# Beryl2000/SE-UNet-AirSeg

Hardware: AMD Instinct MI355X
Metric: voxels/sec SE-UNet fwd+bwd, 128^3 patch (higher is better)
Workload: dtype bf16

## Files before the change

### include/seunet_hip.h

```cpp
#ifndef SEUNET_HIP_H
#define SEUNET_HIP_H
#include <stddef.h>

#ifdef __cplusplus
extern "C" {
#endif

#ifndef SEUNET_F32
#define SEUNET_F32 0
#define SEUNET_BF16 1
#define SEUNET_F16 2
#endif
#define SEUNET_CONV_MFMA 0
#define SEUNET_CONV_NAIVE 1
#define SEUNET_CONV_MARCH 2
#define SEUNET_CONV_TILED 3

typedef void* seunet_stream_t;
typedef struct seunet_dims { int n, d, h, w; } seunet_dims;

int seunet_version(void);
const char* seunet_last_error(void);
int seunet_init(int device);

int seunet_pack_cl(int dtype, const float* in_ncdhw, int c, void* out_cl, int c_pad, seunet_dims dims, seunet_stream_t s);
int seunet_unpack_cl(int dtype, const void* in_cl, int c, float* out_ncdhw, seunet_dims dims, seunet_stream_t s);

size_t seunet_conv_wpack_bytes(int dtype, int taps, int cin, int cout);
int seunet_conv_pack_weights(int dtype, const float* w, int taps, int cin, int cout, int transpose_flip, void* wpack, seunet_stream_t s);
int seunet_conv_stats_slots(int impl, int taps, int dilation, seunet_dims dims);
int seunet_conv3d_fwd(int dtype, int impl, int taps, int dilation, int nsrc, const void* const* src, const int* src_c,
                      int cin, const void* weights, int transpose_flip, const float* bias, int ndst, void* const* dst,
                      const int* dst_c, const int* dst_accumulate, double* stats_partial, seunet_dims dims, seunet_stream_t s);
int seunet_conv3d_stream_supported(int dtype, int dilation, int src_c, int dst_c);
size_t seunet_conv3d_stream_wpack_bytes(int src_c);
int seunet_conv3d_stream_slots(int dilation, seunet_dims dims);
int seunet_conv3d_stream_pack(int dtype, const float* w, int cin_w, int cout_w, int transpose_flip, int src_c, int dst_c, void* wpack,
                              seunet_stream_t s);
int seunet_conv3d_stream(int dtype, int dilation, const void* src, int src_c, const void* wpack, const float* bias, void* dst, int dst_c,
                         int dst_accumulate, double* stats_partial, seunet_dims dims, seunet_stream_t s);
int seunet_conv3d_march_supported(int dtype, int dilation, int nsrc, const int* src_c, int ndst, const int* dst_c);
size_t seunet_conv3d_march_wpack_bytes(int cin, int cout);
int seunet_conv3d_march_slots(int dilation, int cin, int cout, seunet_dims dims);
int seunet_conv3d_march_pack(int dtype, const float* w, int cin_w, int cout_w, int transpose_flip, int cin, int cout, void* wpack,
                             seunet_stream_t s);
int seunet_conv3d_march(int dtype, int dilation, int nsrc, const void* const* src, const int* src_c, const void* wpack, const float* bias,
                        int ndst, void* const* dst, const int* dst_c, const int* dst_accumulate, double* stats_partial, seunet_dims dims,
                        seunet_stream_t s);
int seunet_conv3d_wgrad_stream_supported(int dtype, int dilation, int x_c, int dy_c);
size_t seunet_conv3d_wgrad_stream_workspace_bytes(int x_c, int dy_c, int dilation, seunet_dims dims);
int seunet_conv3d_wgrad_stream(int dtype, int dilation, const void* x, int x_c, int cin, const void* dy, int dy_c, int cout, float* dw,
                               void* workspace, size_t workspace_bytes, seunet_dims dims, seunet_stream_t s);
size_t seunet_conv3d_wgrad_workspace_bytes(int taps, int cin, int cout);
int seunet_conv3d_wgrad(int dtype, int impl, int taps, int dilation, int nsrc, const void* const* src, const int* src_c,
                        int cin, const void* dy, int cout, float* dw, void* workspace, size_t workspace_bytes,
                        seunet_dims dims, seunet_stream_t s);

int seunet_epilogue_slots(seunet_dims dims);
int seunet_channel_stats(int dtype, const void* t, int c, double* partial, seunet_dims dims, seunet_stream_t s);
int seunet_stats_finalize(const double* partial, int slots, int c, int n, long long count, float eps, int mode,
                          float* out_a, float* out_b, seunet_stream_t s);

int seunet_gate_epilogue_fwd(int dtype, const void* raw, const float* mean, const float* rstd, int c, const float* w_se,
                             const float* w_se2, const float* w_side, const float* b_side, float slope, void* e_out,
                             float* side_out, float* level_map, int level_accumulate, const float* head_w,
                             const float* drop, int drop_stride, seunet_dims dims, seunet_stream_t s);
int seunet_gate_epilogue_bwd(int dtype, const void* raw, const float* mean, const float* rstd, int c, const float* w_se,
                             const float* w_se2, const float* w_side, const float* b_side, float slope, const void* g_e,
                             const float* g_side, const float* g_level, const float* head_w, const float* drop,
                             int drop_stride, const float* m1, const float* m2, void* draw_out, double* stat_partial,
                             float* pgrad_partial, seunet_dims dims, seunet_stream_t s);
int seunet_pgrad_reduce(const float* pgrad_partial, int records, int c, float* dw_se, float* dw_se2, float* dw_side,
                        float* db_side, float* dhead_w, seunet_stream_t s);
int seunet_gate_bwd_finalize(const double* stat_partial, int slots, int c, int n, long long count, float* m1, float* m2,
                             const float* pgrad_partial, int records, float* dw_se, float* dw_se2, float* dw_side,
                             float* db_side, float* dhead_w, seunet_stream_t s);

int seunet_cat_epilogue_fwd(int dtype, const void* raw, const float* mean, const float* rstd, const void* raw2,
                            const float* mean2, const float* rstd2, int c, float slope, void* out, seunet_dims dims,
                            seunet_stream_t s);
int seunet_cat_epilogue_bwd(int dtype, const void* g_out, const void* raw, const float* mean, const float* rstd,
                            const void* raw2, const float* mean2, const float* rstd2, int c, float slope,
                            const float* m1, const float* m2, const float* m1b, const float* m2b, void* dx, void* dx2,
                            double* stat_partial, double* stat_partial2, seunet_dims dims, seunet_stream_t s);

int seunet_xbranch_moment_slots(seunet_dims dims);
int seunet_xbranch_moments(int dtype, const void* x_in, double* partial , seunet_dims dims, seunet_stream_t s);
int seunet_xbranch_stats(const double* partial, int slots, const float* w2, int c, int in_channel, int n, long long count,
                         float eps, float* mean2, float* rstd2, double* moments_out , seunet_stream_t s);
int seunet_cat_epilogue_fwd_x(int dtype, const void* raw, const float* mean, const float* rstd, const void* x_in,
                              const float* w2, int in_channel, const float* mean2, const float* rstd2, int c, float slope,
                              void* out, seunet_dims dims, seunet_stream_t s);
int seunet_cat_epilogue_bwd_x(int dtype, const void* g_out, const void* raw, const float* mean, const float* rstd,
                              const void* x_in, const float* w2, int in_channel, const float* mean2, const float* rstd2,
                              int c, float slope, const float* m1, const float* m2, const float* m1b, const float* m2b,
                              void* dx, double* stat_partial, double* stat_partial2, double* xw_partial, seunet_dims dims,
                              seunet_stream_t s);
int seunet_cat_epilogue_fwd_x_pool(int dtype, const void* raw, const float* mean, const float* rstd, const void* x_in,
                                   const float* w2, int in_channel, const float* mean2, const float* rstd2, int c, float slope,
                                   void* out, void* pooled, unsigned int* argmax, seunet_dims dims, seunet_stream_t s);
int seunet_cat_epilogue_bwd_x_pool(int dtype, const void* g_out, const void* raw, const float* mean, const float* rstd,
                                   const void* x_in, const float* w2, int in_channel, const float* mean2, const float* rstd2,
                                   int c, float slope, const float* m1, const float* m2, const float* m1b, const float* m2b,
                                   void* dx, double* stat_partial, double* stat_partial2, double* xw_partial,
                                   const unsigned int* pool_argmax, const void* pool_g, seunet_dims dims, seunet_stream_t s);
int seunet_cat_xgrad_finalize(const double* xw_partial, const double* stat_partial2, int slots, const double* moments,
                              const float* w2, int c, int in_channel, int n, float eps, float* dw, seunet_stream_t s);

int seunet_maxpool_fwd(int dtype, const void* in, int c, void* out, seunet_dims in_dims, seunet_stream_t s);
int seunet_maxpool_bwd(int dtype, const void* in, const void* g_out, int c, void* g_in, int accumulate,
                       seunet_dims in_dims, seunet_stream_t s);
int seunet_upsample2_fwd(int dtype, const void* in, int c, void* out, seunet_dims in_dims, seunet_stream_t s);
int seunet_upsample2_bwd(int dtype, const void* g_out, int c, void* g_in, int accumulate, seunet_dims in_dims,
                         seunet_stream_t s);
int seunet_side_upsample(const float* side, int c, int scale, float* out_ncdhw, int c_total, int c_off,
                         seunet_dims low_dims, seunet_stream_t s);

int seunet_head_fwd(const float* const* level_maps, int nlevels, const float* bias, float* pred, seunet_dims dims,
                    seunet_stream_t s);
size_t seunet_head_bwd_tmp_floats(seunet_dims dims);
int seunet_head_bwd(const float* g_pred, float* const* g_levels, int nlevels, float* tmp, float* g_bias,
                    seunet_dims dims, seunet_stream_t s);

#define SEUNET_LOSS_DICE 1
#define SEUNET_LOSS_GUL 2
#define SEUNET_LOSS_ATR 4
int seunet_loss_partial_floats(void);
int seunet_loss_sums(const float* pred, int apply_sigmoid, const float* target, const float* weight, const float* skel,
                     long long n, float* partial, double* sums, int terms, seunet_stream_t s);
int seunet_loss_value(const double* sums0, double c_dice0, double c_gul0, double c_atr0, const double* sums1, double c_dice1,
                      double c_gul1, double c_atr1, float* value, seunet_stream_t s);
int seunet_loss_grad(const float* pred, int apply_sigmoid, const float* target, const float* weight, const float* skel,
                     long long n, const double* sums, float c_dice, float c_gul, float c_atr, float g_scale,
                     const float* g_scale_dev, float* g_pred, seunet_stream_t s);

int seunet_loss_sample_partial_floats(int batch);
int seunet_loss_sums_per_sample(const float* pred, int apply_sigmoid, const float* target, const float* weight, const float* skel,
                                int batch, long long n_per_sample, float* partial, double* sums, int terms, seunet_stream_t s);
int seunet_loss_sample_values(const double* sums, int batch, double c_dice, double c_gul, double c_atr, float* values,
                              seunet_stream_t s);

int seunet_pool_select(const float* new_keys, int batch, float* keys, long long* seq, long long* state, int capacity, int* slots_out,
                       seunet_stream_t s);
int seunet_pool_scatter(const int* slots_dev, int batch, int capacity, long long voxels, const float* data, const float* label,
                        const float* weight, const float* skel, float* pool_data, unsigned char* pool_label, float* pool_weight,
                        unsigned char* pool_skel, seunet_stream_t s);
int seunet_pool_gather(const int* slots_host, int n, int capacity, long long voxels, const float* pool_data,
                       const unsigned char* pool_label, const float* pool_weight, const unsigned char* pool_skel, float* data_out,
                       float* label_out, float* weight_out, float* skel_out, seunet_stream_t s);

int seunet_adamw_step(float* const* params, const float* const* grads, float* const* exp_avg, float* const* exp_avg_sq,
                      const long long* counts, int n_tensors, double lr, double beta1, double beta2, double eps,
                      double weight_decay, int step, int maximize, seunet_stream_t s);

#define SEUNET_IMG_I16 0
#define SEUNET_IMG_F32 1
#define SEUNET_W_F16 0
#define SEUNET_W_F32 1
#define SEUNET_W_F64 2
int seunet_crop_batch(const void* img, int img_dtype, const unsigned char* label, const void* weight, int weight_dtype,
                      const unsigned char* skeleton, int d, int h, int w, int cube, int ncrop, const int* starts, const int* aug,
                      double weight_exponent, int f64_math, float* data_out, float* label_out, float* weight_out, float* skel_out,
                      seunet_stream_t s);
int seunet_hu_two_channel(const void* img, int img_dtype, long long nvox, int f64_math, float* out, seunet_stream_t s);

int seunet_window_gather(const float* volume, int c, int x, int y, int z, int cube, int nwin, const int* starts, float* out,
                         seunet_stream_t s);
int seunet_window_accumulate(const float* logits, int apply_sigmoid, int nwin, const int* starts, int cube, double* acc, int x, int y,
                             int z, seunet_stream_t s);
int seunet_window_finalize(const double* acc, int x, int y, int z, int cube, int nx, const int* xs, int ny, const int* ys, int nz,
                           const int* zs, int dup0, double* out, seunet_stream_t s);

#define SEUNET_DTI_F64 0
#define SEUNET_DTI_F32 1
size_t seunet_dti_workspace_bytes(int h, int w, int z);
int seunet_dti(const double* pred, int h, int w, int z, double h_thresh, double l_thresh, int pred_dtype, unsigned char* out,
               void* workspace, size_t workspace_bytes, seunet_stream_t s);

#define SEUNET_CC_EVALUATION 0
#define SEUNET_CC_MAXIMUM_3D 1
#define SEUNET_CC_LARGEST_FILLED 2
size_t seunet_cc_workspace_bytes(int h, int w, int z);
int seunet_largest_component(const unsigned char* volume, int h, int w, int z, int rule, unsigned char* out, int* status_dev,
                             void* workspace, size_t workspace_bytes, seunet_stream_t s);
size_t seunet_metric_out_bytes(int nbins);
int seunet_metric_sums(const unsigned char* pred, const unsigned char* label, const unsigned char* skeleton, const int* parsing,
                       long long n, int nbins, void* out, size_t out_bytes, seunet_stream_t s);

size_t seunet_edt_workspace_bytes(int n0, int n1, int n2);
int seunet_edt(const unsigned char* volume, int n0, int n1, int n2, int* sqdist, double* dist, int* indices, int* status_dev,
               void* workspace, size_t workspace_bytes, seunet_stream_t s);
int seunet_mask_bits(const unsigned char* mask, long long n, unsigned long long* bits, seunet_stream_t s);
int seunet_hard_mining_masks(const unsigned char* label, const unsigned char* skeleton, const unsigned char* pred, int n0, int n1,
                             int n2, unsigned long long* skeleton_bits, unsigned long long* small_bits, seunet_stream_t s);
size_t seunet_lib_weight_workspace_bytes(int n0, int n1, int n2);
int seunet_lib_weight(const unsigned char* label, int n0, int n1, int n2, const float* table, void* out, void* workspace,
                      size_t workspace_bytes, seunet_stream_t s);
size_t seunet_break_weight_workspace_bytes(int n0, int n1, int n2);
int seunet_break_weight(const unsigned char* label, const unsigned char* pred, const unsigned char* skeleton, int n0, int n1, int n2,
                        void* w_br, unsigned char* br_skel, int* status_dev, void* workspace, size_t workspace_bytes,
                        seunet_stream_t s);

size_t seunet_skeleton_workspace_bytes(int n0, int n1, int n2);
int seunet_skeletonize(const unsigned char* volume, int n0, int n1, int n2, unsigned char* out, int* passes_dev, void* workspace,
                       size_t workspace_bytes, seunet_stream_t s);

size_t seunet_skeleton_branches_workspace_bytes(int n0, int n1, int n2);
int seunet_skeleton_branches(const unsigned char* skeleton, int n0, int n1, int n2, int min_voxels, int* cd, unsigned char* skeleton_parse,
                             int* num_dev, void* workspace, size_t workspace_bytes, seunet_stream_t s);
size_t seunet_parse_assign_workspace_bytes(int n0, int n1, int n2);
int seunet_parse_assign(const unsigned char* skeleton_parse, const int* cd, const unsigned char* label, int n0, int n1, int n2,
                        int* parsing, int* status_dev, void* workspace, size_t workspace_bytes, seunet_stream_t s);
int seunet_label_stats_max_num(void);
int seunet_label_stats(const int* parsing, int n0, int n1, int n2, int num, unsigned int* counts, unsigned long long* adjacency_bits,
                       int* status_dev, seunet_stream_t s);
int seunet_relabel(const int* parsing, long long n, const int* lut, int nlut, int* out, seunet_stream_t s);

#define SEUNET_MORPH_DILATE 0
#define SEUNET_MORPH_ERODE_BORDER0 1
#define SEUNET_MORPH_ERODE_BORDER1 2
#define SEUNET_MORPH_CLOSE 3
size_t seunet_binary_morph_workspace_bytes(int n0, int n1, int n2);
int seunet_binary_morph(const unsigned char* volume, int n0, int n1, int n2, int op, unsigned char* out, void* workspace,
                        size_t workspace_bytes, seunet_stream_t s);
int seunet_fill_holes(const unsigned char* volume, int n0, int n1, int n2, unsigned char* out, void* workspace, size_t workspace_bytes,
                      seunet_stream_t s);
int seunet_slice_moments(const unsigned char* mask, int n0, int n1, int n2, int k, unsigned long long* out_dev, seunet_stream_t s);
int seunet_scatter_labels(const long long* lin_index_dev, const int* value_dev, long long m, long long n, int* cd,
                          unsigned char* skeleton_parse, int* status_dev, seunet_stream_t s);

size_t seunet_mesh_workspace_bytes(int n0, int n1, int n2);
int seunet_mesh_count(const unsigned char* volume, int n0, int n1, int n2, long long* nverts, long long* nfaces, void* workspace,
                      size_t workspace_bytes, seunet_stream_t s);
int seunet_mesh_emit(int n0, int n1, int n2, double level, long long nverts, long long nfaces, float* verts, int* faces,
                     const void* workspace, size_t workspace_bytes, seunet_stream_t s);
int seunet_mesh_coord_sums(const unsigned char* mask, int n0, int n1, int n2, long long* sums_dev, seunet_stream_t s);
size_t seunet_mesh_adjacency_workspace_bytes(long long nverts, long long nfaces);
int seunet_mesh_adjacency(const int* faces, long long nfaces, long long nverts, int* indptr, int* indices, long long indices_capacity,
                          unsigned char* boundary, int* status_dev, void* workspace, size_t workspace_bytes, seunet_stream_t s);
int seunet_mesh_smooth(const float* verts, long long nverts, const int* indptr, const int* indices, const unsigned char* boundary,
                       int n_iter, float relaxation_factor, float* out, float* tmp, seunet_stream_t s);
int seunet_mesh_affine(const float* verts, long long nverts, const float* centre, const float* scale, float* out, seunet_stream_t s);
int seunet_mesh_stl_records(const float* verts, long long nverts, const int* faces, long long nfaces, const float* centre,
                            const float* scale, unsigned char* records, int* status_dev, seunet_stream_t s);

int seunet_value_counts(const short* ct, long long n, int shift, unsigned int* counts, seunet_stream_t s);
int seunet_shift_clamp(const short* ct, long long n, int shift, int clamp, int clamp_le, int clamp_to, short* out, seunet_stream_t s);
size_t seunet_get_l_workspace_bytes(int h, int w, int z);
int seunet_get_l(const short* ct, int h, int w, int z, double T, int min_area, unsigned char* out, void* workspace,
                 size_t workspace_bytes, seunet_stream_t s);
int seunet_mask_combine(const unsigned char* a, const unsigned char* b, long long n, int op, unsigned char* out, seunet_stream_t s);
int seunet_mask_box(const unsigned char* mask, int h, int w, int z, int* box_dev, seunet_stream_t s);
int seunet_crop3d(const void* src, int elem_bytes, int h, int w, int z, const int* box, void* dst, seunet_stream_t s);

typedef struct seunet_net_desc {
  int batch, in_channel, n_classes;
  int d, h, w;
  int width_mult;
  int dtype;
  int conv_impl;
  float negative_slope;
  float eps;
} seunet_net_desc;

int seunet_net_param_count(const seunet_net_desc* desc);
int seunet_net_param_info(const seunet_net_desc* desc, int index, char* name, int name_cap, int* shape5, int* ndim);
size_t seunet_net_workspace_bytes(const seunet_net_desc* desc);
int seunet_net_forward(const seunet_net_desc* desc, const float* const* params, const float* x, const float* drop1,
                       const float* drop2, float* pred0, float* pred1, void* workspace, size_t workspace_bytes,
                       seunet_stream_t s);
int seunet_net_forward_capture(const seunet_net_desc* desc, const float* const* params, const float* x, const float* drop1,
                               const float* drop2, float* pred0, float* pred1, void* workspace, size_t workspace_bytes,
                               seunet_stream_t s, void** graph_out);
int seunet_graph_launch(void* graph, seunet_stream_t s);
int seunet_graph_destroy(void* graph);
int seunet_net_read_tensor(const seunet_net_desc* desc, const float* const* params, const void* workspace, size_t workspace_bytes,
                           const char* name, int which, float* out, int* channels, seunet_stream_t s);
#define SEUNET_KERNEL_NAIVE 0
#define SEUNET_KERNEL_TILED 1
#define SEUNET_KERNEL_STREAM 2
#define SEUNET_KERNEL_MARCH 3
#define SEUNET_KERNEL_WGRAD1X1 4
typedef struct seunet_conv_info {
  char name[16];
  int taps, dilation, level;
  seunet_dims dims;
  int nsrc, src_c[3], src_is_input[3];
  int cin, cout;
  int need_dgrad;
  int fwd, dgrad, wgrad;
  char x_name[16];
  int x_materialised, x_fwd, x_wgrad;
  long long src_dist;
} seunet_conv_info;
int seunet_net_conv_info(const seunet_net_desc* desc, int index, seunet_conv_info* out);
int seunet_net_backward(const seunet_net_desc* desc, const float* const* params, const float* g_pred0,
                        const float* g_pred1, const float* drop1, const float* drop2, float* const* grads,
                        void* workspace, size_t workspace_bytes, seunet_stream_t s);
int seunet_net_backward_ev(const seunet_net_desc* desc, const float* const* params, const float* g_pred0,
                           const float* g_pred1, const float* drop1, const float* drop2, float* const* grads,
                           void* workspace, size_t workspace_bytes, seunet_stream_t s, void* decoder_done_event);
size_t seunet_net_input_grad_bytes(const seunet_net_desc* desc);
int seunet_net_backward_input(const seunet_net_desc* desc, const float* const* params, const float* g_pred0,
                              const float* g_pred1, const float* drop1, const float* drop2, float* const* grads, float* grad_x,
                              void* scratch, size_t scratch_bytes, void* workspace, size_t workspace_bytes, seunet_stream_t s,
                              void* decoder_done_event);

int seunet_prof_enable(int on);
int seunet_prof_enable_filtered(const char* tag_substring);
int seunet_prof_report(char* buf, size_t cap);

#ifdef __cplusplus
}
#endif
#endif
```

### se-unet-airseg_amd/_lib.py

```python
from __future__ import annotations

import ctypes as C
import os
from typing import Optional, Sequence

_HERE = os.path.dirname(os.path.abspath(__file__))
LIB_PATH = os.environ.get("SEUNET_LIB") or os.path.join(_HERE, "libseunet_hip.so")

F32, BF16, F16 = 0, 1, 2
CONV_MFMA, CONV_NAIVE, CONV_MARCH, CONV_TILED = 0, 1, 2, 3
LOSS_NSUMS = 7
DTI_F64, DTI_F32 = 0, 1
CC_EVALUATION, CC_MAXIMUM_3D, CC_LARGEST_FILLED = 0, 1, 2
MORPH_DILATE, MORPH_ERODE_BORDER0, MORPH_ERODE_BORDER1, MORPH_CLOSE = 0, 1, 2, 3


class Dims(C.Structure):
    _fields_ = [("n", C.c_int), ("d", C.c_int), ("h", C.c_int), ("w", C.c_int)]


class NetDesc(C.Structure):
    _fields_ = [("batch", C.c_int), ("in_channel", C.c_int), ("n_classes", C.c_int),
                ("d", C.c_int), ("h", C.c_int), ("w", C.c_int), ("width_mult", C.c_int),
                ("dtype", C.c_int), ("conv_impl", C.c_int),
                ("negative_slope", C.c_float), ("eps", C.c_float)]


KERNEL_NAIVE, KERNEL_TILED, KERNEL_STREAM, KERNEL_MARCH, KERNEL_WGRAD1X1 = range(5)
KERNEL_NAMES = ("Naive", "Tiled", "Stream", "March", "Wgrad1x1")


class ConvInfo(C.Structure):
    _fields_ = [("name", C.c_char * 16), ("taps", C.c_int), ("dilation", C.c_int), ("level", C.c_int), ("dims", Dims),
                ("nsrc", C.c_int), ("src_c", C.c_int * 3), ("src_is_input", C.c_int * 3), ("cin", C.c_int), ("cout", C.c_int),
                ("need_dgrad", C.c_int), ("fwd", C.c_int), ("dgrad", C.c_int), ("wgrad", C.c_int),
                ("x_name", C.c_char * 16), ("x_materialised", C.c_int), ("x_fwd", C.c_int), ("x_wgrad", C.c_int),
                ("src_dist", C.c_longlong)]


_vp, _i, _f, _ll, _sz, _d =C.c_void_p, C.c_int, C.c_float, C.c_longlong, C.c_size_t, C.c_double
_pp = C.POINTER(C.c_void_p)
_ip = C.POINTER(C.c_int)

PROTOTYPES = {
    "seunet_version": (_i, []),
    "seunet_last_error": (C.c_char_p, []),
    "seunet_pack_cl": (_i, [_i, _vp, _i, _vp, _i, Dims, _vp]),
    "seunet_unpack_cl": (_i, [_i, _vp, _i, _vp, Dims, _vp]),
    "seunet_conv_wpack_bytes": (_sz, [_i, _i, _i, _i]),
    "seunet_conv_pack_weights": (_i, [_i, _vp, _i, _i, _i, _i, _vp, _vp]),
    "seunet_conv_stats_slots": (_i, [_i, _i, _i, Dims]),
    "seunet_conv3d_fwd": (_i, [_i, _i, _i, _i, _i, _pp, _ip, _i, _vp, _i, _vp, _i, _pp, _ip, _ip, _vp, Dims, _vp]),
    "seunet_conv3d_stream_supported": (_i, [_i, _i, _i, _i]),
    "seunet_conv3d_stream_wpack_bytes": (_sz, [_i]),
    "seunet_conv3d_stream_slots": (_i, [_i, Dims]),
    "seunet_conv3d_stream_pack": (_i, [_i, _vp, _i, _i, _i, _i, _i, _vp, _vp]),
    "seunet_conv3d_stream": (_i, [_i, _i, _vp, _i, _vp, _vp, _vp, _i, _i, _vp, Dims, _vp]),
    "seunet_conv3d_march_supported": (_i, [_i, _i, _i, _ip, _i, _ip]),
    "seunet_conv3d_march_wpack_bytes": (_sz, [_i, _i]),
    "seunet_conv3d_march_slots": (_i, [_i, _i, _i, Dims]),
    "seunet_conv3d_march_pack": (_i, [_i, _vp, _i, _i, _i, _i, _i, _vp, _vp]),
    "seunet_conv3d_march": (_i, [_i, _i, _i, _pp, _ip, _vp, _vp, _i, _pp, _ip, _ip, _vp, Dims, _vp]),
    "seunet_conv3d_wgrad_stream_supported": (_i, [_i, _i, _i, _i]),
    "seunet_conv3d_wgrad_stream_workspace_bytes": (_sz, [_i, _i, _i, Dims]),
    "seunet_conv3d_wgrad_stream": (_i, [_i, _i, _vp, _i, _i, _vp, _i, _i, _vp, _vp, _sz, Dims, _vp]),
    "seunet_conv3d_wgrad_workspace_bytes": (_sz, [_i, _i, _i]),
    "seunet_conv3d_wgrad": (_i, [_i, _i, _i, _i, _i, _pp, _ip, _i, _vp, _i, _vp, _vp, _sz, Dims, _vp]),
    "seunet_epilogue_slots": (_i, [Dims]),
    "seunet_channel_stats": (_i, [_i, _vp, _i, _vp, Dims, _vp]),
    "seunet_stats_finalize": (_i, [_vp, _i, _i, _i, _ll, _f, _i, _vp, _vp, _vp]),
    "seunet_gate_epilogue_fwd": (_i, [_i, _vp, _vp, _vp, _i, _vp, _vp, _vp, _vp, _f, _vp, _vp, _vp, _i, _vp, _vp, _i, Dims, _vp]),
    "seunet_gate_epilogue_bwd": (_i, [_i, _vp, _vp, _vp, _i, _vp, _vp, _vp, _vp, _f, _vp, _vp, _vp, _vp, _vp, _i, _vp, _vp, _vp, _vp, _vp, Dims, _vp]),
    "seunet_pgrad_reduce": (_i, [_vp, _i, _i, _vp, _vp, _vp, _vp, _vp, _vp]),
    "seunet_gate_bwd_finalize": (_i, [_vp, _i, _i, _i, _ll, _vp, _vp, _vp, _i, _vp, _vp, _vp, _vp, _vp, _vp]),
    "seunet_cat_epilogue_fwd": (_i, [_i, _vp, _vp, _vp, _vp, _vp, _vp, _i, _f, _vp, Dims, _vp]),
    "seunet_cat_epilogue_bwd": (_i, [_i, _vp, _vp, _vp, _vp, _vp, _vp, _vp, _i, _f, _vp, _vp, _vp, _vp, _vp, _vp, _vp, _vp, Dims, _vp]),
    "seunet_maxpool_fwd": (_i, [_i, _vp, _i, _vp, Dims, _vp]),
    "seunet_maxpool_bwd": (_i, [_i, _vp, _vp, _i, _vp, _i, Dims, _vp]),
    "seunet_upsample2_fwd": (_i, [_i, _vp, _i, _vp, Dims, _vp]),
    "seunet_upsample2_bwd": (_i, [_i, _vp, _i, _vp, _i, Dims, _vp]),
    "seunet_side_upsample": (_i, [_vp, _i, _i, _vp, _i, _i, Dims, _vp]),
    "seunet_head_fwd": (_i, [_pp, _i, _vp, _vp, Dims, _vp]),
    "seunet_head_bwd_tmp_floats": (_sz, [Dims]),
    "seunet_head_bwd": (_i, [_vp, _pp, _i, _vp, _vp, Dims, _vp]),
    "seunet_loss_partial_floats": (_i, []),
    "seunet_loss_sums": (_i, [_vp, _i, _vp, _vp, _vp, _ll, _vp, _vp, _i, _vp]),
    "seunet_loss_value": (_i, [_vp, _d, _d, _d, _vp, _d, _d, _d, _vp, _vp]),
    "seunet_loss_grad": (_i, [_vp, _i, _vp, _vp, _vp, _ll, _vp, _f, _f, _f, _f, _vp, _vp, _vp]),
    "seunet_loss_sample_partial_floats": (_i, [_i]),
    "seunet_loss_sums_per_sample": (_i, [_vp, _i, _vp, _vp, _vp, _i, _ll, _vp, _vp, _i, _vp]),
    "seunet_loss_sample_values": (_i, [_vp, _i, _d, _d, _d, _vp, _vp]),
    "seunet_pool_select": (_i, [_vp, _i, _vp, _vp, _vp, _i, _vp, _vp]),
    "seunet_pool_scatter": (_i, [_vp, _i, _i, _ll, _vp, _vp, _vp, _vp, _vp, _vp, _vp, _vp, _vp]),
    "seunet_pool_gather": (_i, [_ip, _i, _i, _ll, _vp, _vp, _vp, _vp, _vp, _vp, _vp, _vp, _vp]),
    "seunet_xbranch_moment_slots": (_i, [Dims]),
    "seunet_xbranch_moments": (_i, [_i, _vp, _vp, Dims, _vp]),
    "seunet_xbranch_stats": (_i, [_vp, _i, _vp, _i, _i, _i, _ll, _f, _vp, _vp, _vp, _vp]),
    "seunet_cat_epilogue_fwd_x": (_i, [_i, _vp, _vp, _vp, _vp, _vp, _i, _vp, _vp, _i, _f, _vp, Dims, _vp]),
    "seunet_cat_epilogue_bwd_x": (_i, [_i, _vp, _vp, _vp, _vp, _vp, _vp, _i, _vp, _vp, _i, _f, _vp, _vp, _vp, _vp, _vp, _vp, _vp, _vp, Dims, _vp]),
    "seunet_cat_epilogue_fwd_x_pool": (_i, [_i, _vp, _vp, _vp, _vp, _vp, _i, _vp, _vp, _i, _f, _vp, _vp, _vp, Dims, _vp]),
    "seunet_cat_epilogue_bwd_x_pool": (_i, [_i, _vp, _vp, _vp, _vp, _vp, _vp, _i, _vp, _vp, _i, _f, _vp, _vp, _vp, _vp, _vp, _vp, _vp, _vp, _vp, _vp, Dims, _vp]),
    "seunet_cat_xgrad_finalize": (_i, [_vp, _vp, _i, _vp, _vp, _i, _i, _i, _f, _vp, _vp]),
    "seunet_cc_workspace_bytes": (_sz, [_i, _i, _i]),
    "seunet_largest_component": (_i, [_vp, _i, _i, _i, _i, _vp, _vp, _vp, _sz, _vp]),
    "seunet_metric_out_bytes": (_sz, [_i]),
    "seunet_metric_sums": (_i, [_vp, _vp, _vp, _vp, _ll, _i, _vp, _sz, _vp]),
    "seunet_value_counts": (_i, [_vp, _ll, _i, _vp, _vp]),
    "seunet_shift_clamp": (_i, [_vp, _ll, _i, _i, _i, _i, _vp, _vp]),
    "seunet_get_l_workspace_bytes": (_sz, [_i, _i, _i]),
    "seunet_get_l": (_i, [_vp, _i, _i, _i, _d, _i, _vp, _vp, _sz, _vp]),
    "seunet_mask_combine": (_i, [_vp, _vp, _ll, _i, _vp, _vp]),
    "seunet_mask_box": (_i, [_vp, _i, _i, _i, _vp, _vp]),
    "seunet_crop3d": (_i, [_vp, _i, _i, _i, _i, _ip, _vp, _vp]),
    "seunet_crop_batch": (_i, [_vp, _i, _vp, _vp, _i, _vp, _i, _i, _i, _i, _i, _ip, _ip, C.c_double, _i, _vp, _vp, _vp, _vp, _vp]),
    "seunet_hu_two_channel": (_i, [_vp, _i, _ll, _i, _vp, _vp]),
    "seunet_window_gather": (_i, [_vp, _i, _i, _i, _i, _i, _i, _ip, _vp, _vp]),
    "seunet_window_accumulate": (_i, [_vp, _i, _i, _ip, _i, _vp, _i, _i, _i, _vp]),
    "seunet_window_finalize": (_i, [_vp, _i, _i, _i, _i, _i, _ip, _i, _ip, _i, _ip, _i, _vp, _vp]),
    "seunet_dti_workspace_bytes": (_sz, [_i, _i, _i]),
    "seunet_dti": (_i, [_vp, _i, _i, _i, C.c_double, C.c_double, _i, _vp, _vp, _sz, _vp]),
    "seunet_edt_workspace_bytes": (_sz, [_i, _i, _i]),
    "seunet_edt": (_i, [_vp, _i, _i, _i, _vp, _vp, _vp, _vp, _vp, _sz, _vp]),
    "seunet_mask_bits": (_i, [_vp, _ll, _vp, _vp]),
    "seunet_hard_mining_masks": (_i, [_vp, _vp, _vp, _i, _i, _i, _vp, _vp, _vp]),
    "seunet_lib_weight_workspace_bytes": (_sz, [_i, _i, _i]),
    "seunet_lib_weight": (_i, [_vp, _i, _i, _i, _vp, _vp, _vp, _sz, _vp]),
    "seunet_break_weight_workspace_bytes": (_sz, [_i, _i, _i]),
    "seunet_break_weight": (_i, [_vp, _vp, _vp, _i, _i, _i, _vp, _vp, _vp, _vp, _sz, _vp]),
    "seunet_skeleton_workspace_bytes": (_sz, [_i, _i, _i]),
    "seunet_skeletonize": (_i, [_vp, _i, _i, _i, _vp, _vp, _vp, _sz, _vp]),
    "seunet_skeleton_branches_workspace_bytes": (_sz, [_i, _i, _i]),
    "seunet_skeleton_branches": (_i, [_vp, _i, _i, _i, _i, _vp, _vp, _vp, _vp, _sz, _vp]),
    "seunet_parse_assign_workspace_bytes": (_sz, [_i, _i, _i]),
    "seunet_parse_assign": (_i, [_vp, _vp, _vp, _i, _i, _i, _vp, _vp, _vp, _sz, _vp]),
    "seunet_label_stats_max_num": (_i, []),
    "seunet_label_stats": (_i, [_vp, _i, _i, _i, _i, _vp, _vp, _vp, _vp]),
    "seunet_relabel": (_i, [_vp, _ll, _vp, _i, _vp, _vp]),
    "seunet_binary_morph_workspace_bytes": (_sz, [_i, _i, _i]),
    "seunet_binary_morph": (_i, [_vp, _i, _i, _i, _i, _vp, _vp, _sz, _vp]),
    "seunet_fill_holes": (_i, [_vp, _i, _i, _i, _vp, _vp, _sz, _vp]),
    "seunet_slice_moments": (_i, [_vp, _i, _i, _i, _i, _vp, _vp]),
    "seunet_scatter_labels": (_i, [_vp, _vp, _ll, _ll, _vp, _vp, _vp, _vp]),
    "seunet_mesh_workspace_bytes": (_sz, [_i, _i, _i]),
    "seunet_mesh_count": (_i, [_vp, _i, _i, _i, C.POINTER(_ll), C.POINTER(_ll), _vp, _sz, _vp]),
    "seunet_mesh_emit": (_i, [_i, _i, _i, _d, _ll, _ll, _vp, _vp, _vp, _sz, _vp]),
    "seunet_mesh_coord_sums": (_i, [_vp, _i, _i, _i, _vp, _vp]),
    "seunet_mesh_adjacency_workspace_bytes": (_sz, [_ll, _ll]),
    "seunet_mesh_adjacency": (_i, [_vp, _ll, _ll, _vp, _vp, _ll, _vp, _vp, _vp, _sz, _vp]),
    "seunet_mesh_smooth": (_i, [_vp, _ll, _vp, _vp, _vp, _i, _f, _vp, _vp, _vp]),
    "seunet_mesh_affine": (_i, [_vp, _ll, C.POINTER(_f), C.POINTER(_f), _vp, _vp]),
    "seunet_mesh_stl_records": (_i, [_vp, _ll, _vp, _ll, C.POINTER(_f), C.POINTER(_f), _vp, _vp, _vp]),
    "seunet_adamw_step": (_i, [_vp, _vp, _vp, _vp, _vp, _i, C.c_double, C.c_double, C.c_double, C.c_double, C.c_double, _i, _i, _vp]),
    "seunet_net_param_count": (_i, [C.POINTER(NetDesc)]),
    "seunet_net_param_info": (_i, [C.POINTER(NetDesc), _i, C.c_char_p, _i, _ip, _ip]),
    "seunet_net_workspace_bytes": (_sz, [C.POINTER(NetDesc)]),
    "seunet_net_forward": (_i, [C.POINTER(NetDesc), _pp, _vp, _vp, _vp, _vp, _vp, _vp, _sz, _vp]),
    "seunet_prof_enable": (_i, [_i]),
    "seunet_prof_enable_filtered": (_i, [C.c_char_p]),
    "seunet_prof_report": (_i, [C.c_char_p, _sz]),
    "seunet_init": (_i, [_i]),
    "seunet_net_forward_capture": (_i, [C.POINTER(NetDesc), _pp, _vp, _vp, _vp, _vp, _vp, _vp, _sz, _vp, C.POINTER(C.c_void_p)]),
    "seunet_graph_launch": (_i, [_vp, _vp]),
    "seunet_graph_destroy": (_i, [_vp]),
    "seunet_net_read_tensor": (_i, [C.POINTER(NetDesc), _pp, _vp, _sz, C.c_char_p, _i, _vp, _ip, _vp]),
    "seunet_net_conv_info": (_i, [C.POINTER(NetDesc), _i, C.POINTER(ConvInfo)]),
    "seunet_net_backward": (_i, [C.POINTER(NetDesc), _pp, _vp, _vp, _vp, _vp, _pp, _vp, _sz, _vp]),
    "seunet_net_backward_ev": (_i, [C.POINTER(NetDesc), _pp, _vp, _vp, _vp, _vp, _pp, _vp, _sz, _vp, _vp]),
    "seunet_net_input_grad_bytes": (_sz, [C.POINTER(NetDesc)]),
    "seunet_net_backward_input": (_i, [C.POINTER(NetDesc), _pp, _vp, _vp, _vp, _vp, _pp, _vp, _vp, _sz, _vp, _sz, _vp, _vp]),
}

_lib: Optional[C.CDLL] = None


def load() -> C.CDLL:
    global _lib
    if _lib is not None:
        return _lib
    if not os.path.exists(LIB_PATH):
        raise RuntimeError(
            f"{LIB_PATH} is missing: build it with `python -c 'import __graft_entry__ as g; g.build()'` "
            "(or `make -C se-unet-airseg_amd/csrc`).  There is no CPU or PyTorch fallback for the HIP path.")
    lib = C.CDLL(LIB_PATH)
    for name, (res, args) in PROTOTYPES.items():
        fn = getattr(lib, name)
        fn.restype, fn.argtypes = res, args
    _lib = lib
    return lib


def last_error() -> str:
    return load().seunet_last_error().decode(errors="replace")


def check(status: int, what: str = "") -> None:
    if status != 0:
        raise RuntimeError(f"libseunet_hip {what}: {last_error()}")


def ptr(t) -> Optional[int]:
    return None if t is None else t.data_ptr()


def ptr_array(tensors: Sequence) -> C.Array:
    arr = (C.c_void_p * len(tensors))()
    for i, t in enumerate(tensors):
        arr[i] = None if t is None else (t if isinstance(t, int) else t.data_ptr())
    return arr


def int_array(vals: Sequence[int]) -> C.Array:
    return (C.c_int * len(vals))(*vals)


def stream_ptr() -> int:
    import torch
    return torch.cuda.current_stream().cuda_stream


def dtype_code(name: str) -> int:
    name = str(name).lower().replace("torch.", "")
    if name in ("bf16", "bfloat16"):
        return BF16
    if name in ("fp32", "f32", "float32", "float"):
        return F32
    if name in ("fp16", "f16", "float16", "half"):
        return F16
    raise ValueError(f"unsupported activation dtype {name!r} (fp32, bf16 or fp16)")
```

### se-unet-airseg_amd/csrc/abi.cpp

```cpp
#include "seunet_common.h"
#include "epilogue.h"
#include "volume.h"
#include "../../include/seunet_hip.h"

using namespace seunet;

static inline Dims D(seunet_dims d) { return Dims{d.n, d.d, d.h, d.w}; }
static inline hipStream_t S(seunet_stream_t s) { return reinterpret_cast<hipStream_t>(s); }

static int make_src(int nsrc, const void* const* src, const int* src_c, SrcList& l) {
  SEUNET_CHECK(nsrc >= 1 && nsrc <= 3 && src && src_c, "bad source list");
  l = SrcList{};
  l.n = nsrc;
  for (int i = 0; i < nsrc; ++i) { l.ptr[i] = src[i]; l.C[i] = src_c[i]; }
  return 0;
}

namespace seunet { extern unsigned long long* g_conv_debug; }

extern "C" {

int seunet_debug_set_buffer(void* p) { seunet::g_conv_debug = reinterpret_cast<unsigned long long*>(p); return 0; }
int seunet_debug_upsample2_form(int dtype, int c, seunet_dims dims, int backward) { return upsample2_form(dtype, c, D(dims), backward != 0); }

int seunet_debug_volume_layout(int op, int n0, int n1, int n2, size_t* offsets, int cap) {
  if (n0 < 1 || n1 < 1 || n2 < 1) return 0;
  size_t at[16];
  WsCarver c(nullptr);
  c.log = at;
  c.log_cap = 16;
  switch (op) {
    case 0: cc_ws(c, n0, n1, n2); break;
    case 1: get_l_ws(c, n0, n1, n2); break;
    case 2: case 8: edt_ws(c, n0, n1, n2); break;
    case 3: lib_weight_ws(c, n0, n1, n2); break;
    case 4: break_weight_ws(c, n0, n1, n2); break;
    case 5: branches_ws(c, n0, n1, n2); break;
    case 6: dti_ws(c, n0, n1, n2); break;
    case 7: if (!skeleton_ws(c, n0, n1, n2)) return 0; break;
    case 9: morph_ws(c, n0, n1, n2); break;
    case 10: if ((long long)n0 * n1 * n2 >= (1ll << 31)) return 0; mesh_ws(c, n0, n1, n2); break;
    default: return -1;
  }
  if (c.taken > c.log_cap) return -1;
  for (int i = 0; i < c.taken && i < cap && offsets; ++i) {
    offsets[2 * i] = at[i];
    offsets[2 * i + 1] = (i + 1 < c.taken ? at[i + 1] : c.bytes()) - at[i];
  }
  return c.taken;
}

int seunet_version(void) { return 201; }
const char* seunet_last_error(void) { return get_error(); }

int seunet_init(int device) {
  int count = 0, prev = 0;
  SEUNET_HIP(hipGetDeviceCount(&count));
  SEUNET_CHECK(device >= 0 && device < count, "init: device %d out of range (%d visible)", device, count);
  SEUNET_HIP(hipGetDevice(&prev));
  SEUNET_HIP(hipSetDevice(device));
  const void* page = seunet::device_zero_page();
  (void)hipSetDevice(prev);
  SEUNET_CHECK(page != nullptr, "init: could not allocate the zero page on device %d", device);
  return 0;
}

int seunet_pack_cl(int dtype, const float* in, int c, void* out, int c_pad, seunet_dims dims, seunet_stream_t s) {
  SEUNET_CHECK(in && out, "pack_cl: null tensor");
  return launch_pack_cl(dtype, in, c, out, c_pad, D(dims), S(s));
}
int seunet_unpack_cl(int dtype, const void* in, int c, float* out, seunet_dims dims, seunet_stream_t s) {
  SEUNET_CHECK(in && out, "unpack_cl: null tensor");
  return launch_unpack_cl(dtype, in, c, out, D(dims), S(s));
}

size_t seunet_conv_wpack_bytes(int dtype, int taps, int cin, int cout) { return conv_wpack_bytes(dtype, taps, cin, cout); }
int seunet_conv_pack_weights(int dtype, const float* w, int taps, int cin, int cout, int tflip, void* wpack, seunet_stream_t s) {
  SEUNET_CHECK(w && wpack, "conv_pack_weights: null tensor");
  return launch_conv_pack_weights(dtype, w, taps, cin, cout, tflip, wpack, S(s));
}
int seunet_conv_stats_slots(int impl, int taps, int dilation, seunet_dims dims) {
  return impl == SEUNET_CONV_NAIVE ? epi_partials(D(dims)) : conv_stats_tiles(D(dims), taps, dilation);
}
int seunet_conv3d_fwd(int dtype, int impl, int taps, int dilation, int nsrc, const void* const* src, const int* src_c, int cin,
                      const void* weights, int tflip, const float* bias, int ndst, void* const* dst, const int* dst_c,
                      const int* dst_acc, double* stats_partial, seunet_dims dims, seunet_stream_t s) {
  SrcList sl;
  if (int e = make_src(nsrc, src, src_c, sl)) return e;
  SEUNET_CHECK(ndst >= 1 && ndst <= 3 && dst && dst_c && weights, "conv3d_fwd: bad destination list / weights");
  DstList dl{};
  dl.n = ndst;
  for (int i = 0; i < ndst; ++i) { dl.ptr[i] = dst[i]; dl.C[i] = dst_c[i]; dl.acc[i] = dst_acc ? dst_acc[i] : 0; }
  if (impl == SEUNET_CONV_NAIVE) {
    if (int e = launch_conv_naive(dtype, taps, dilation, sl, cin, (const float*)weights, tflip, bias, dl, D(dims), S(s))) return e;
    if (stats_partial) {
      SEUNET_CHECK(ndst == 1, "conv3d_fwd: statistics need a single destination");
      return launch_channel_stats(dtype, dst[0], dst_c[0], stats_partial, D(dims), S(s));
    }
    return 0;
  }
  return launch_conv_igemm(dtype, taps, dilation, sl, cin, weights, bias, dl, stats_partial, D(dims), S(s));
}
int seunet_conv3d_stream_supported(int dtype, int dilation, int src_c, int dst_c) { return conv_stream_supported(dtype, 27, dilation, src_c, dst_c) ? 1 : 0; }
size_t seunet_conv3d_stream_wpack_bytes(int src_c) { return conv_stream_wpack_bytes(src_c); }
int seunet_conv3d_stream_slots(int dilation, seunet_dims dims) { return conv_stream_slots(D(dims), dilation); }
int seunet_conv3d_stream_pack(int dtype, const float* w, int cin_w, int cout_w, int transpose_flip, int src_c, int dst_c, void* wpack,
                              seunet_stream_t s) {
  return launch_conv_stream_pack(dtype, w, cin_w, cout_w, transpose_flip, src_c, dst_c, wpack, S(s));
}
int seunet_conv3d_stream(int dtype, int dilation, const void* src, int src_c, const void* wpack, const float* bias, void* dst, int dst_c,
                         int dst_accumulate, double* stats_partial, seunet_dims dims, seunet_stream_t s) {
  return launch_conv_stream(dtype, dilation, src, src_c, wpack, bias, dst, dst_c, dst_accumulate, stats_partial, D(dims), S(s));
}
static int make_dst(int ndst, void* const* dst, const int* dst_c, const int* dst_acc, DstList& dl) {
  SEUNET_CHECK(ndst >= 1 && ndst <= 3 && dst_c, "bad destination list");
  dl = DstList{};
  dl.n = ndst;
  for (int i = 0; i < ndst; ++i) { dl.ptr[i] = dst ? dst[i] : nullptr; dl.C[i] = dst_c[i]; dl.acc[i] = dst_acc ? dst_acc[i] : 0; }
  return 0;
}
int seunet_conv3d_march_supported(int dtype, int dilation, int nsrc, const int* src_c, int ndst, const int* dst_c) {
  if (nsrc < 1 || nsrc > 3 || ndst < 1 || ndst > 3 || !src_c || !dst_c) return 0;
  SrcList sl{}; DstList dl{};
  sl.n = nsrc; dl.n = ndst;
  for (int i = 0; i < nsrc; ++i) sl.C[i] = src_c[i];
  for (int i = 0; i < ndst; ++i) dl.C[i] = dst_c[i];
  return conv_march_supported(dtype, 27, dilation, sl, dl) ? 1 : 0;
}
size_t seunet_conv3d_march_wpack_bytes(int cin, int cout) { return conv_march_wpack_bytes(cin, cout); }
int seunet_conv3d_march_slots(int dilation, int cin, int cout, seunet_dims dims) { return conv_march_slots(D(dims), dilation, cin, cout); }
int seunet_conv3d_march_pack(int dtype, const float* w, int cin_w, int cout_w, int transpose_flip, int cin, int cout, void* wpack,
                             seunet_stream_t s) {
  return launch_conv_march_pack(dtype, w, cin_w, cout_w, transpose_flip, cin, cout, wpack, S(s));
}
int seunet_conv3d_march(int dtype, int dilation, int nsrc, const void* const* src, const int* src_c, const void* wpack, const float* bias,
                        int ndst, void* const* dst, const int* dst_c, const int* dst_accumulate, double* stats_partial, seunet_dims dims,
                        seunet_stream_t s) {
  SrcList sl; DstList dl;
  if (int e = make_src(nsrc, src, src_c, sl)) return e;
  SEUNET_CHECK(dst != nullptr, "conv3d_march: null destination list");
  if (int e = make_dst(ndst, dst, dst_c, dst_accumulate, dl)) return e;
  return launch_conv_march(dtype, dilation, sl, wpack, bias, dl, stats_partial, D(dims), S(s));
}
int seunet_conv3d_wgrad_stream_supported(int dtype, int dilation, int x_c, int dy_c) { return wgrad_stream_supported(dtype, 27, dilation, x_c, dy_c) ? 1 : 0; }
size_t seunet_conv3d_wgrad_stream_workspace_bytes(int x_c, int dy_c, int dilation, seunet_dims dims) {
  return wgrad_stream_workspace_bytes(x_c, dy_c, dilation, D(dims));
}
int seunet_conv3d_wgrad_stream(int dtype, int dilation, const void* x, int x_c, int cin, const void* dy, int dy_c, int cout, float* dw,
                               void* workspace, size_t workspace_bytes, seunet_dims dims, seunet_stream_t s) {
  return launch_wgrad_stream(dtype, dilation, x, x_c, cin, dy, dy_c, cout, dw, workspace, workspace_bytes, D(dims), S(s));
}
size_t seunet_conv3d_wgrad_workspace_bytes(int taps, int cin, int cout) { return wgrad_workspace_bytes(taps, cin, cout); }
int seunet_conv3d_wgrad(int dtype, int impl, int taps, int dilation, int nsrc, const void* const* src, const int* src_c, int cin,
                        const void* dy, int cout, float* dw, void* workspace, size_t workspace_bytes, seunet_dims dims,
                        seunet_stream_t s) {
  SrcList sl;
  if (int e = make_src(nsrc, src, src_c, sl)) return e;
  SEUNET_CHECK(dy && dw, "conv3d_wgrad: null tensor");
  if (impl == SEUNET_CONV_NAIVE) return launch_wgrad_naive(dtype, taps, dilation, sl, cin, dy, cout, dw, D(dims), S(s));
  SEUNET_CHECK(workspace, "conv3d_wgrad: null workspace");
  const ConvKernel k = impl == SEUNET_CONV_MARCH ? (taps == 1 ? ConvKernel::Wgrad1x1 : ConvKernel::March)
                       : impl == SEUNET_CONV_TILED ? ConvKernel::Tiled
                                                   : wgrad_kernel(dtype, taps, dilation, sl, cin, cout, D(dims), sl.gap());
  return run_wgrad(k, dtype, taps, dilation, sl, cin, dy, cout, dw, workspace, workspace_bytes, D(dims), S(s));
}

int seunet_epilogue_slots(seunet_dims dims) { return epi_partials(D(dims)); }
int seunet_channel_stats(int dtype, const void* t, int c, double* partial, seunet_dims dims, seunet_stream_t s) {
  SEUNET_CHECK(t && partial, "channel_stats: null tensor");
  return launch_channel_stats(dtype, t, c, partial, D(dims), S(s));
}
int seunet_stats_finalize(const double* partial, int slots, int c, int n, long long count, float eps, int mode, float* out_a,
                          float* out_b, seunet_stream_t s) {
  SEUNET_CHECK(partial && out_a && out_b && slots >= 1 && count >= 1, "stats_finalize: bad argument");
  return launch_stats_finalize(partial, slots, c, n, count, eps, mode, out_a, out_b, S(s));
}

int seunet_gate_epilogue_fwd(int dtype, const void* raw, const float* mean, const float* rstd, int c, const float* w_se,
                             const float* w_se2, const float* w_side, const float* b_side, float slope, void* e_out,
                             float* side_out, float* level_map, int level_accumulate, const float* head_w, const float* drop,
                             int drop_stride, seunet_dims dims, seunet_stream_t s) {
  SEUNET_CHECK(raw && mean && rstd && w_se && w_side && b_side && e_out, "gate_epilogue_fwd: null tensor");
  SEUNET_CHECK(!level_map || head_w, "gate_epilogue_fwd: level_map needs head_w");
  const GateBlock b{{raw, mean, rstd}, c, {w_se, w_se2, w_side, b_side, slope}};
  SseHead h{side_out, level_map, level_accumulate, head_w, drop, drop_stride};
  return launch_sse_fwd(dtype, b, e_out, h, D(dims), S(s));
}
int seunet_gate_epilogue_bwd(int dtype, const void* raw, const float* mean, const float* rstd, int c, const float* w_se,
                             const float* w_se2, const float* w_side, const float* b_side, float slope, const void* g_e,
                             const float* g_side, const float* g_level, const float* head_w, const float* drop, int drop_stride,
                             const float* m1, const float* m2, void* draw_out, double* stat_partial, float* pgrad_partial,
                             seunet_dims dims, seunet_stream_t s) {
  SEUNET_CHECK(raw && mean && rstd && w_se && w_side && b_side, "gate_epilogue_bwd: null tensor");
  SEUNET_CHECK(!g_level || head_w, "gate_epilogue_bwd: g_level needs head_w");
  const GateBlock b{{raw, mean, rstd}, c, {w_se, w_se2, w_side, b_side, slope}};
  SseBwdIn g{g_e, g_side, g_level};
  SseHead h{nullptr, nullptr, 0, head_w, drop, drop_stride};
  if (m1 == nullptr) return launch_sse_bwd_sums(dtype, b, g, h, {stat_partial, pgrad_partial}, D(dims), S(s));
  return launch_sse_bwd_apply(dtype, b, g, h, {m1, m2, draw_out}, D(dims), S(s));
}
int seunet_pgrad_reduce(const float* pgrad_partial, int records, int c, float* dw_se, float* dw_se2, float* dw_side,
                        float* db_side, float* dhead_w, seunet_stream_t s) {
  SEUNET_CHECK(pgrad_partial && records >= 1, "pgrad_reduce: bad argument");
  return launch_pgrad_reduce(pgrad_partial, records, c, dw_se, dw_se2, dw_side, db_side, dhead_w, S(s));
}
int seunet_gate_bwd_finalize(const double* stat_partial, int slots, int c, int n, long long count, float* m1, float* m2,
                             const float* pgrad_partial, int records, float* dw_se, float* dw_se2, float* dw_side,
                             float* db_side, float* dhead_w, seunet_stream_t s) {
  SEUNET_CHECK(stat_partial && m1 && m2 && pgrad_partial && slots >= 1 && n >= 1 && count >= 1, "gate_bwd_finalize: bad argument");
  SEUNET_CHECK(c % 8 == 0 && c >= 8 && c <= 128 && (c & (c - 1)) == 0, "channel count %d must be a power of two in [8,128]", c);
  SEUNET_CHECK(records == n * slots, "gate_bwd_finalize: records=%d, pass A wrote n * slots = %d", records, n * slots);
  return launch_gate_bwd_finalize(stat_partial, slots, c, n, count, m1, m2, pgrad_partial, records, dw_se, dw_se2, dw_side,
                                  db_side, dhead_w, S(s));
}
static int cat_epilogue_bwd(int dtype, const CatBlock& b, const void* g_out, const PoolGrad& pool, const float* m1, const float* m2,
                            const float* m1b, const float* m2b, void* dx, void* dx2, double* stat_partial, double* stat_partial2,
                            double* xw_partial, seunet_dims dims, seunet_stream_t s) {
  if (m1 == nullptr) return launch_cat_bwd_sums(dtype, b, g_out, pool, {stat_partial, stat_partial2, xw_partial}, D(dims), S(s));
  return launch_cat_bwd_apply(dtype, b, g_out, pool, {m1, m2, m1b, m2b, dx, dx2, nullptr, 0}, D(dims), S(s));
}
int seunet_cat_epilogue_fwd(int dtype, const void* raw, const float* mean, const float* rstd, const void* raw2,
                            const float* mean2, const float* rstd2, int c, float slope, void* out, seunet_dims dims,
                            seunet_stream_t s) {
  SEUNET_CHECK(raw && mean && rstd && out && (!raw2 || (mean2 && rstd2)), "cat_epilogue_fwd: null tensor");
  const CatBlock b{{raw, mean, rstd}, {raw2 ? Branch2::Stored : Branch2::None, raw2, mean2, rstd2, nullptr, 0}, c, slope};
  return launch_cat_fwd(dtype, b, out, PoolOut{}, D(dims), S(s));
}
int seunet_cat_epilogue_bwd(int dtype, const void* g_out, const void* raw, const float* mean, const float* rstd,
                            const void* raw2, const float* mean2, const float* rstd2, int c, float slope, const float* m1,
                            const float* m2, const float* m1b, const float* m2b, void* dx, void* dx2, double* stat_partial,
                            double* stat_partial2, seunet_dims dims, seunet_stream_t s) {
  SEUNET_CHECK(g_out && raw && mean && rstd, "cat_epilogue_bwd: null tensor");
  SEUNET_CHECK(!raw2 || (mean2 && rstd2), "cat_epilogue_bwd: second branch incomplete");
  const CatBlock b{{raw, mean, rstd}, {raw2 ? Branch2::Stored : Branch2::None, raw2, mean2, rstd2, nullptr, 0}, c, slope};
  return cat_epilogue_bwd(dtype, b, g_out, PoolGrad{}, m1, m2, m1b, m2b, dx, dx2, stat_partial, stat_partial2, nullptr, dims, s);
}

int seunet_maxpool_fwd(int dtype, const void* in, int c, void* out, seunet_dims d, seunet_stream_t s) {
  SEUNET_CHECK(in && out, "maxpool_fwd: null tensor");
  return launch_maxpool_fwd(dtype, in, c, out, D(d), S(s));
}
int seunet_maxpool_bwd(int dtype, const void* in, const void* g_out, int c, void* g_in, int accumulate, seunet_dims d,
                       seunet_stream_t s) {
  SEUNET_CHECK(in && g_out && g_in, "maxpool_bwd: null tensor");
  return launch_maxpool_bwd(dtype, in, g_out, c, g_in, accumulate, D(d), S(s));
}
int seunet_upsample2_fwd(int dtype, const void* in, int c, void* out, seunet_dims d, seunet_stream_t s) {
  SEUNET_CHECK(in && out, "upsample2_fwd: null tensor");
  return launch_upsample2_fwd(dtype, in, c, out, D(d), S(s));
}
int seunet_upsample2_bwd(int dtype, const void* g_out, int c, void* g_in, int accumulate, seunet_dims d, seunet_stream_t s) {
  SEUNET_CHECK(g_out && g_in, "upsample2_bwd: null tensor");
  return launch_upsample2_bwd(dtype, g_out, c, g_in, accumulate, D(d), S(s));
}
int seunet_side_upsample(const float* side, int c, int scale, float* out, int c_total, int c_off, seunet_dims low,
                         seunet_stream_t s) {
  SEUNET_CHECK(side && out && scale >= 1, "side_upsample: bad argument");
  return launch_side_upsample(side, c, scale, out, c_total, c_off, D(low), S(s));
}

int seunet_head_fwd(const float* const* level_maps, int nlevels, const float* bias, float* pred, seunet_dims d, seunet_stream_t s) {
  SEUNET_CHECK(level_maps && bias && pred, "head_fwd: null tensor");
  return launch_head_fwd(level_maps, nlevels, bias, pred, D(d), S(s));
}
size_t seunet_head_bwd_tmp_floats(seunet_dims d) { return head_bwd_tmp_floats(D(d)); }
int seunet_head_bwd(const float* g_pred, float* const* g_levels, int nlevels, float* tmp, float* g_bias, seunet_dims d,
                    seunet_stream_t s) {
  SEUNET_CHECK(g_pred && g_levels && tmp, "head_bwd: null tensor");
  return launch_head_bwd(g_pred, g_levels, nlevels, tmp, g_bias, D(d), S(s));
}

int seunet_loss_partial_floats(void) { return loss_partials() * SEUNET_LOSS_NSUMS; }
int seunet_loss_sums(const float* pred, int apply_sigmoid, const float* target, const float* weight, const float* skel,
                     long long n, float* partial, double* sums, int terms, seunet_stream_t s) {
  SEUNET_CHECK(pred && target && partial && sums && n >= 1, "loss_sums: bad argument");
  SEUNET_CHECK(terms >= 0 && terms <= 7, "loss_sums: terms=%d is not a mask of SEUNET_LOSS_DICE | _GUL | _ATR", terms);
  return launch_loss_sums(pred, apply_sigmoid, target, weight, skel, n, partial, sums, S(s), terms);
}
int seunet_loss_value(const double* sums0, double c_dice0, double c_gul0, double c_atr0, const double* sums1, double c_dice1,
                      double c_gul1, double c_atr1, float* value, seunet_stream_t s) {
  SEUNET_CHECK(sums0 && value, "loss_value: null argument");
  return launch_loss_value(sums0, c_dice0, c_gul0, c_atr0, sums1, c_dice1, c_gul1, c_atr1, value, S(s));
}
int seunet_loss_grad(const float* pred, int apply_sigmoid, const float* target, const float* weight, const float* skel,
                     long long n, const double* sums, float c_dice, float c_gul, float c_atr, float g_scale,
                     const float* g_scale_dev, float* g_pred, seunet_stream_t s) {
  SEUNET_CHECK(pred && target && sums && g_pred && n >= 1, "loss_grad: bad argument");
  return launch_loss_grad(pred, apply_sigmoid, target, weight, skel, n, sums, c_dice, c_gul, c_atr, g_scale, g_scale_dev, g_pred, S(s));
}

int seunet_loss_sample_partial_floats(int batch) {
  if (batch < 1 || batch > 65535) { fail("loss_sample_partial_floats: batch %d (1..65535)", batch); return 0; }
  return loss_sample_partials(batch) * SEUNET_LOSS_NSUMS;
}
int seunet_loss_sums_per_sample(const float* pred, int apply_sigmoid, const float* target, const float* weight, const float* skel,
                                int batch, long long n_per_sample, float* partial, double* sums, int terms, seunet_stream_t s) {
  SEUNET_CHECK(pred && target && partial && sums && n_per_sample >= 1, "loss_sums_per_sample: bad argument");
  SEUNET_CHECK(batch >= 1 && batch <= 65535, "loss_sums_per_sample: batch %d (1..65535)", batch);
  SEUNET_CHECK(terms >= 0 && terms <= 7, "loss_sums_per_sample: terms=%d is not a mask of SEUNET_LOSS_DICE | _GUL | _ATR", terms);
  return launch_loss_sums_per_sample(pred, apply_sigmoid, target, weight, skel, batch, n_per_sample, partial, sums, terms, S(s));
}
int seunet_loss_sample_values(const double* sums, int batch, double c_dice, double c_gul, double c_atr, float* values, seunet_stream_t s) {
  SEUNET_CHECK(sums && values && batch >= 1, "loss_sample_values: bad argument");
  return launch_loss_sample_values(sums, batch, c_dice, c_gul, c_atr, values, S(s));
}

int seunet_pool_select(const float* new_keys, int batch, float* keys, long long* seq, long long* state, int capacity, int* slots_out,
                       seunet_stream_t s) {
  return launch_pool_select(new_keys, batch, keys, seq, state, capacity, slots_out, S(s));
}
int seunet_pool_scatter(const int* slots_dev, int batch, int capacity, long long voxels, const float* data, const float* label,
                        const float* weight, const float* skel, float* pool_data, unsigned char* pool_label, float* pool_weight,
                        unsigned char* pool_skel, seunet_stream_t s) {
  return launch_pool_scatter(slots_dev, batch, capacity, voxels, data, label, weight, skel, pool_data, pool_label, pool_weight, pool_skel,
                             S(s));
}
int seunet_pool_gather(const int* slots_host, int n, int capacity, long long voxels, const float* pool_data,
                       const unsigned char* pool_label, const float* pool_weight, const unsigned char* pool_skel, float* data_out,
                       float* label_out, float* weight_out, float* skel_out, seunet_stream_t s) {
  return launch_pool_gather(slots_host, n, capacity, voxels, pool_data, pool_label, pool_weight, pool_skel, data_out, label_out,
                            weight_out, skel_out, S(s));
}

int seunet_xbranch_moment_slots(seunet_dims dims) { return xbranch_moment_slots(D(dims)); }
int seunet_xbranch_moments(int dtype, const void* x_in, double* partial, seunet_dims dims, seunet_stream_t s) {
  SEUNET_CHECK(x_in && partial, "xbranch_moments: null argument");
  return launch_xbranch_moments(dtype, x_in, partial, D(dims), S(s));
}
int seunet_xbranch_stats(const double* partial, int slots, const float* w2, int c, int in_channel, int n, long long count,
                         float eps, float* mean2, float* rstd2, double* moments_out, seunet_stream_t s) {
  SEUNET_CHECK(partial && w2 && mean2 && rstd2 && slots >= 1 && c >= 1 && n >= 1 && count >= 1, "xbranch_stats: bad argument");
  return launch_xbranch_stats(partial, slots, w2, c, in_channel, n, count, eps, mean2, rstd2, moments_out, S(s));
}
int seunet_cat_epilogue_fwd_x(int dtype, const void* raw, const float* mean, const float* rstd, const void* x_in,
                              const float* w2, int in_channel, const float* mean2, const float* rstd2, int c, float slope,
                              void* out, seunet_dims dims, seunet_stream_t s) {
  SEUNET_CHECK(raw && mean && rstd && x_in && w2 && mean2 && rstd2 && out, "cat_epilogue_fwd_x: null argument");
  const CatBlock b{{raw, mean, rstd}, {Branch2::Recomputed, x_in, mean2, rstd2, w2, in_channel}, c, slope};
  return launch_cat_fwd(dtype, b, out, PoolOut{}, D(dims), S(s));
}
int seunet_cat_epilogue_bwd_x(int dtype, const void* g_out, const void* raw, const float* mean, const float* rstd,
                              const void* x_in, const float* w2, int in_channel, const float* mean2, const float* rstd2,
                              int c, float slope, const float* m1, const float* m2, const float* m1b, const float* m2b,
                              void* dx, double* stat_partial, double* stat_partial2, double* xw_partial, seunet_dims dims,
                              seunet_stream_t s) {
  SEUNET_CHECK(g_out && raw && mean && rstd && x_in && w2 && mean2 && rstd2, "cat_epilogue_bwd_x: null argument");
  const CatBlock b{{raw, mean, rstd}, {Branch2::Recomputed, x_in, mean2, rstd2, w2, in_channel}, c, slope};
  return cat_epilogue_bwd(dtype, b, g_out, PoolGrad{}, m1, m2, m1b, m2b, dx, nullptr, stat_partial, stat_partial2, xw_partial, dims, s);
}
int seunet_cat_epilogue_fwd_x_pool(int dtype, const void* raw, const float* mean, const float* rstd, const void* x_in,
                                   const float* w2, int in_channel, const float* mean2, const float* rstd2, int c, float slope,
                                   void* out, void* pooled, unsigned int* argmax, seunet_dims dims, seunet_stream_t s) {
  SEUNET_CHECK(raw && mean && rstd && x_in && w2 && mean2 && rstd2 && out && pooled, "cat_epilogue_fwd_x_pool: null argument");
  const CatBlock b{{raw, mean, rstd}, {Branch2::Recomputed, x_in, mean2, rstd2, w2, in_channel}, c, slope};
  return launch_cat_fwd(dtype, b, out, PoolOut{pooled, argmax}, D(dims), S(s));
}
int seunet_cat_epilogue_bwd_x_pool(int dtype, const void* g_out, const void* raw, const float* mean, const float* rstd,
                                   const void* x_in, const float* w2, int in_channel, const float* mean2, const float* rstd2,
                                   int c, float slope, const float* m1, const float* m2, const float* m1b, const float* m2b,
                                   void* dx, double* stat_partial, double* stat_partial2, double* xw_partial,
                                   const unsigned int* pool_argmax, const void* pool_g, seunet_dims dims, seunet_stream_t s) {
  SEUNET_CHECK(g_out && raw && mean && rstd && x_in && w2 && mean2 && rstd2, "cat_epilogue_bwd_x_pool: null argument");
  SEUNET_CHECK((pool_argmax == nullptr) == (pool_g == nullptr), "cat_epilogue_bwd_x_pool: pool_argmax and pool_g go together");
  const CatBlock b{{raw, mean, rstd}, {Branch2::Recomputed, x_in, mean2, rstd2, w2, in_channel}, c, slope};
  return cat_epilogue_bwd(dtype, b, g_out, PoolGrad{pool_argmax, pool_g}, m1, m2, m1b, m2b, dx, nullptr, stat_partial, stat_partial2,
                          xw_partial, dims, s);
}
int seunet_cat_xgrad_finalize(const double* xw_partial, const double* stat_partial2, int slots, const double* moments, const float* w2,
                              int c, int in_channel, int n, float eps, float* dw, seunet_stream_t s) {
  SEUNET_CHECK(xw_partial && stat_partial2 && moments && w2 && dw && slots >= 1 && c >= 8 && n >= 1, "cat_xgrad_finalize: bad argument");
  return launch_cat_xgrad_finalize(xw_partial, stat_partial2, slots, moments, w2, c, in_channel, n, eps, dw, S(s));
}

size_t seunet_cc_workspace_bytes(int h, int w, int z) {
  if (h < 1 || w < 1 || z < 1) { fail("cc_workspace_bytes: bad dimensions"); return 0; }
  return cc_workspace_bytes(h, w, z);
}
int seunet_largest_component(const unsigned char* volume, int h, int w, int z, int rule, unsigned char* out, int* status_dev,
                             void* workspace, size_t workspace_bytes, seunet_stream_t s) {
  return launch_largest_component(volume, h, w, z, rule, out, status_dev, workspace, workspace_bytes, S(s));
}
size_t seunet_metric_out_bytes(int nbins) { return nbins < 1 ? 0 : metric_out_bytes(nbins); }
int seunet_metric_sums(const unsigned char* pred, const unsigned char* label, const unsigned char* skeleton, const int* parsing,
                       long long n, int nbins, void* out, size_t out_bytes, seunet_stream_t s) {
  return launch_metric_sums(pred, label, skeleton, parsing, n, nbins, out, out_bytes, S(s));
}

size_t seunet_edt_workspace_bytes(int n0, int n1, int n2) {
  if (n0 < 1 || n1 < 1 || n2 < 1) { fail("edt_workspace_bytes: bad dimensions"); return 0; }
  return edt_workspace_bytes(n0, n1, n2);
}
int seunet_edt(const unsigned char* volume, int n0, int n1, int n2, int* sqdist, double* dist, int* indices, int* status_dev,
               void* workspace, size_t workspace_bytes, seunet_stream_t s) {
  return launch_edt(volume, n0, n1, n2, sqdist, dist, indices, status_dev, workspace, workspace_bytes, S(s));
}
int seunet_mask_bits(const unsigned char* mask, long long n, unsigned long long* bits, seunet_stream_t s) {
  return launch_mask_bits(mask, n, bits, S(s));
}
int seunet_hard_mining_masks(const unsigned char* label, const unsigned char* skeleton, const unsigned char* pred, int n0, int n1,
                             int n2, unsigned long long* skeleton_bits, unsigned long long* small_bits, seunet_stream_t s) {
  return launch_hm_candidates(label, skeleton, pred, n0, n1, n2, skeleton_bits, small_bits, S(s));
}
size_t seunet_lib_weight_workspace_bytes(int n0, int n1, int n2) {
  if (n0 < 1 || n1 < 1 || n2 < 1) { fail("lib_weight_workspace_bytes: bad dimensions"); return 0; }
  return lib_weight_workspace_bytes(n0, n1, n2);
}
int seunet_lib_weight(const unsigned char* label, int n0, int n1, int n2, const float* table, void* out, void* workspace,
                      size_t workspace_bytes, seunet_stream_t s) {
  return launch_lib_weight(label, n0, n1, n2, table, out, workspace, workspace_bytes, S(s));
}
size_t seunet_break_weight_workspace_bytes(int n0, int n1, int n2) {
  if (n0 < 1 || n1 < 1 || n2 < 1) { fail("break_weight_workspace_bytes: bad dimensions"); return 0; }
  return break_weight_workspace_bytes(n0, n1, n2);
}
int seunet_break_weight(const unsigned char* label, const unsigned char* pred, const unsigned char* skeleton, int n0, int n1, int n2,
                        void* w_br, unsigned char* br_skel, int* status_dev, void* workspace, size_t workspace_bytes,
                        seunet_stream_t s) {
  return launch_break_weight(label, pred, skeleton, n0, n1, n2, w_br, br_skel, status_dev, workspace, workspace_bytes, S(s));
}

size_t seunet_skeleton_workspace_bytes(int n0, int n1, int n2) {
  const size_t bytes = skeleton_workspace_bytes(n0, n1, n2);
  if (bytes == 0) fail("skeleton_workspace_bytes: bad dimensions (%d, %d, %d): extents >= 1, at most 2^31-1 voxels", n0, n1, n2);
  return bytes;
}
int seunet_skeletonize(const unsigned char* volume, int n0, int n1, int n2, unsigned char* out, int* passes_dev, void* workspace,
                       size_t workspace_bytes, seunet_stream_t s) {
  return launch_skeletonize(volume, n0, n1, n2, out, passes_dev, workspace, workspace_bytes, S(s));
}

size_t seunet_skeleton_branches_workspace_bytes(int n0, int n1, int n2) {
  if (n0 < 1 || n1 < 1 || n2 < 1 || (long long)n0 * n1 * n2 >= (1ll << 31)) { fail("skeleton_branches_workspace_bytes: bad dimensions"); return 0; }
  return skeleton_branches_workspace_bytes(n0, n1, n2);
}
int seunet_skeleton_branches(const unsigned char* skeleton, int n0, int n1, int n2, int min_voxels, int* cd, unsigned char* skeleton_parse,
                             int* num_dev, void* workspace, size_t workspace_bytes, seunet_stream_t s) {
  return launch_skeleton_branches(skeleton, n0, n1, n2, min_voxels, cd, skeleton_parse, num_dev, workspace, workspace_bytes, S(s));
}
size_t seunet_parse_assign_workspace_bytes(int n0, int n1, int n2) {
  if (n0 < 1 || n1 < 1 || n2 < 1) { fail("parse_assign_workspace_bytes: bad dimensions"); return 0; }
  return parse_assign_workspace_bytes(n0, n1, n2);
}
int seunet_parse_assign(const unsigned char* skeleton_parse, const int* cd, const unsigned char* label, int n0, int n1, int n2,
                        int* parsing, int* status_dev, void* workspace, size_t workspace_bytes, seunet_stream_t s) {
  return launch_parse_assign(skeleton_parse, cd, label, n0, n1, n2, parsing, status_dev, workspace, workspace_bytes, S(s));
}
int seunet_label_stats_max_num(void) { return label_stats_max_num(); }
int seunet_label_stats(const int* parsing, int n0, int n1, int n2, int num, unsigned int* counts, unsigned long long* adjacency_bits,
                       int* status_dev, seunet_stream_t s) {
  return launch_label_stats(parsing, n0, n1, n2, num, counts, adjacency_bits, status_dev, S(s));
}
int seunet_relabel(const int* parsing, long long n, const int* lut, int nlut, int* out, seunet_stream_t s) {
  return launch_relabel(parsing, n, lut, nlut, out, S(s));
}

size_t seunet_binary_morph_workspace_bytes(int n0, int n1, int n2) {
  if (n0 < 1 || n1 < 1 || n2 < 1) { fail("binary_morph_workspace_bytes: bad dimensions"); return 0; }
  return binary_morph_workspace_bytes(n0, n1, n2);
}
int seunet_binary_morph(const unsigned char* volume, int n0, int n1, int n2, int op, unsigned char* out, void* workspace,
                        size_t workspace_bytes, seunet_stream_t s) {
  return launch_binary_morph(volume, n0, n1, n2, op, out, workspace, workspace_bytes, S(s));
}
int seunet_fill_holes(const unsigned char* volume, int n0, int n1, int n2, unsigned char* out, void* workspace, size_t workspace_bytes,
                      seunet_stream_t s) {
  return launch_fill_holes(volume, n0, n1, n2, out, workspace, workspace_bytes, S(s));
}
int seunet_slice_moments(const unsigned char* mask, int n0, int n1, int n2, int k, unsigned long long* out_dev, seunet_stream_t s) {
  return launch_slice_moments(mask, n0, n1, n2, k, out_dev, S(s));
}
int seunet_scatter_labels(const long long* lin_index_dev, const int* value_dev, long long m, long long n, int* cd,
                          unsigned char* skeleton_parse, int* status_dev, seunet_stream_t s) {
  return launch_scatter_labels(lin_index_dev, value_dev, m, n, cd, skeleton_parse, status_dev, S(s));
}

size_t seunet_mesh_workspace_bytes(int n0, int n1, int n2) {
  if (volume_check("mesh_workspace_bytes", n0, n1, n2, 0)) return 0;
  return mesh_workspace_bytes(n0, n1, n2);
}
int seunet_mesh_count(const unsigned char* volume, int n0, int n1, int n2, long long* nverts, long long* nfaces, void* workspace,
                      size_t workspace_bytes, seunet_stream_t s) {
  return launch_mesh_count(volume, n0, n1, n2, nverts, nfaces, workspace, workspace_bytes, S(s));
}
int seunet_mesh_emit(int n0, int n1, int n2, double level, long long nverts, long long nfaces, float* verts, int* faces,
                     const void* workspace, size_t workspace_bytes, seunet_stream_t s) {
  return launch_mesh_emit(n0, n1, n2, level, nverts, nfaces, verts, faces, workspace, workspace_bytes, S(s));
}
int seunet_mesh_coord_sums(const unsigned char* mask, int n0, int n1, int n2, long long* sums_dev, seunet_stream_t s) {
  return launch_mesh_coord_sums(mask, n0, n1, n2, sums_dev, S(s));
}
size_t seunet_mesh_adjacency_workspace_bytes(long long nverts, long long nfaces) {
  if (nverts < 0 || nfaces < 0 || nverts > 0x7ffffffell || 6 * nfaces > 0x7fffffffll) {
    fail("mesh_adjacency_workspace_bytes: bad sizes (%lld vertices, %lld faces)", nverts, nfaces);
    return 0;
  }
  return mesh_adjacency_workspace_bytes(nverts, nfaces);
}
int seunet_mesh_adjacency(const int* faces, long long nfaces, long long nverts, int* indptr, int* indices, long long indices_capacity,
                          unsigned char* boundary, int* status_dev, void* workspace, size_t workspace_bytes, seunet_stream_t s) {
  return launch_mesh_adjacency(faces, nfaces, nverts, indptr, indices, indices_capacity, boundary, status_dev, workspace, workspace_bytes,
                               S(s));
}
int seunet_mesh_smooth(const float* verts, long long nverts, const int* indptr, const int* indices, const unsigned char* boundary,
                       int n_iter, float relaxation_factor, float* out, float* tmp, seunet_stream_t s) {
  return launch_mesh_smooth(verts, nverts, indptr, indices, boundary, n_iter, relaxation_factor, out, tmp, S(s));
}
int seunet_mesh_affine(const float* verts, long long nverts, const float* centre, const float* scale, float* out, seunet_stream_t s) {
  return launch_mesh_affine(verts, nverts, centre, scale, out, S(s));
}
int seunet_mesh_stl_records(const float* verts, long long nverts, const int* faces, long long nfaces, const float* centre,
                            const float* scale, unsigned char* records, int* status_dev, seunet_stream_t s) {
  return launch_mesh_stl_records(verts, nverts, faces, nfaces, centre, scale, records, status_dev, S(s));
}

int seunet_value_counts(const short* ct, long long n, int shift, unsigned int* counts, seunet_stream_t s) {
  return launch_value_counts(ct, n, shift, counts, S(s));
}
int seunet_shift_clamp(const short* ct, long long n, int shift, int clamp, int clamp_le, int clamp_to, short* out, seunet_stream_t s) {
  return launch_shift_clamp(ct, n, shift, clamp, clamp_le, clamp_to, out, S(s));
}
size_t seunet_get_l_workspace_bytes(int h, int w, int z) {
  if (h < 1 || w < 1 || z < 1) { fail("get_l_workspace_bytes: bad dimensions"); return 0; }
  return get_l_workspace_bytes(h, w, z);
}
int seunet_get_l(const short* ct, int h, int w, int z, double T, int min_area, unsigned char* out, void* workspace,
                 size_t workspace_bytes, seunet_stream_t s) {
  return launch_get_l(ct, h, w, z, T, min_area, out, workspace, workspace_bytes, S(s));
}
int seunet_mask_combine(const unsigned char* a, const unsigned char* b, long long n, int op, unsigned char* out, seunet_stream_t s) {
  return launch_mask_combine(a, b, n, op, out, S(s));
}
int seunet_mask_box(const unsigned char* mask, int h, int w, int z, int* box_dev, seunet_stream_t s) {
  return launch_mask_box(mask, h, w, z, box_dev, S(s));
}
int seunet_crop3d(const void* src, int elem_bytes, int h, int w, int z, const int* box, void* dst, seunet_stream_t s) {
  return launch_crop3d(src, elem_bytes, h, w, z, box, dst, S(s));
}

int seunet_crop_batch(const void* img, int img_dtype, const unsigned char* label, const void* weight, int weight_dtype,
                      const unsigned char* skeleton, int d, int h, int w, int cube, int ncrop, const int* starts, const int* aug,
                      double weight_exponent, int f64_math, float* data_out, float* label_out, float* weight_out, float* skel_out,
                      seunet_stream_t s) {
  return launch_crop_batch(img, img_dtype, label, weight, weight_dtype, skeleton, d, h, w, cube, ncrop, starts, aug, weight_exponent,
                           f64_math, data_out, label_out, weight_out, skel_out, S(s));
}
int seunet_hu_two_channel(const void* img, int img_dtype, long long nvox, int f64_math, float* out, seunet_stream_t s) {
  return launch_hu_two_channel(img, img_dtype, nvox, f64_math, out, S(s));
}

int seunet_window_gather(const float* volume, int c, int x, int y, int z, int cube, int nwin, const int* starts, float* out,
                         seunet_stream_t s) {
  return launch_window_gather(volume, c, x, y, z, cube, nwin, starts, out, S(s));
}
int seunet_window_accumulate(const float* logits, int apply_sigmoid, int nwin, const int* starts, int cube, double* acc, int x, int y,
                             int z, seunet_stream_t s) {
  return launch_window_accumulate(logits, apply_sigmoid, nwin, starts, cube, acc, x, y, z, S(s));
}
int seunet_window_finalize(const double* acc, int x, int y, int z, int cube, int nx, const int* xs, int ny, const int* ys, int nz,
                           const int* zs, int dup0, double* out, seunet_stream_t s) {
  return launch_window_finalize(acc, x, y, z, cube, nx, xs, ny, ys, nz, zs, dup0, out, S(s));
}

size_t seunet_dti_workspace_bytes(int h, int w, int z) {
  if (h < 1 || w < 1 || z < 1) { fail("dti_workspace_bytes: bad dimensions"); return 0; }
  return dti_workspace_bytes(h, w, z);
}
int seunet_dti(const double* pred, int h, int w, int z, double h_thresh, double l_thresh, int pred_dtype, unsigned char* out,
               void* workspace, size_t workspace_bytes, seunet_stream_t s) {
  return launch_dti(pred, h, w, z, h_thresh, l_thresh, pred_dtype, out, workspace, workspace_bytes, S(s));
}

int seunet_adamw_step(float* const* params, const float* const* grads, float* const* exp_avg, float* const* exp_avg_sq,
                      const long long* counts, int n_tensors, double lr, double beta1, double beta2, double eps,
                      double weight_decay, int step, int maximize, seunet_stream_t s) {
  SEUNET_CHECK(n_tensors == 0 || (params && grads && exp_avg && exp_avg_sq && counts), "adamw_step: bad argument");
  return launch_adamw(params, grads, exp_avg, exp_avg_sq, counts, n_tensors, lr, beta1, beta2, eps, weight_decay, step,
                      maximize, S(s));
}

}
```

### se-unet-airseg_amd/csrc/conv_igemm.hip

```cpp
#include "seunet_common.h"
#include "lds_dma.h"
#include "mfma.h"

namespace seunet {

static constexpr int CV_TZ = 4, CV_TY = 4, CV_TX = 32;

struct ConvKArgs {
  const void* src0; const void* src1; const void* src2;
  int srcC0, srcC1, srcC2;
  int cum1, cum2;
  int cin;
  const void* wpack;
  const float* bias;
  void* dst0; void* dst1; void* dst2;
  int dstC0, dstC1, dstC2;
  int dcum1, dcum2;
  int dacc0, dacc1, dacc2;
  int cout;
  double* stats;
  int N, D, H, W;
  int tx, ty, tz;
  int nchunks;
  int pair;
  int direct;
  int ncb;
  unsigned long long* debug;
};

template <typename T> struct Frag;
template <> struct Frag<bf16_t> { static constexpr int KC = 16, KSTEPS = 1; };
template <> struct Frag<f16_t> { static constexpr int KC = 16, KSTEPS = 1; };
template <> struct Frag<float> { static constexpr int KC = 8, KSTEPS = 4; };

template <int CTRL> __device__ __forceinline__ float xlane_dpp(float v) { return dpp_fetch<CTRL>(v); }
template <int CTRL> __device__ __forceinline__ double xlane_dpp(double v) {
  const unsigned long long u = __builtin_bit_cast(unsigned long long, v);
  const unsigned lo = (unsigned)dpp_fetch_bits<CTRL>((int)(unsigned)u);
  const unsigned hi = (unsigned)dpp_fetch_bits<CTRL>((int)(unsigned)(u >> 32));
  return __builtin_bit_cast(double, ((unsigned long long)hi << 32) | lo);
}
__device__ __forceinline__ float xlane_swz16(float v) {
  return dpp_settle(__builtin_bit_cast(float, __builtin_amdgcn_ds_swizzle(__builtin_bit_cast(int, v), 0x401F)));
}
__device__ __forceinline__ double xlane_swz16(double v) {
  const unsigned long long u = __builtin_bit_cast(unsigned long long, v);
  const unsigned lo = (unsigned)dpp_settle(__builtin_amdgcn_ds_swizzle((int)(unsigned)u, 0x401F));
  const unsigned hi = (unsigned)dpp_settle(__builtin_amdgcn_ds_swizzle((int)(unsigned)(u >> 32), 0x401F));
  return __builtin_bit_cast(double, ((unsigned long long)hi << 32) | lo);
}

#ifdef SEUNET_STAMP
#define STAMP(i) do { const unsigned long long _t = __builtin_readcyclecounter(); ph[i] += _t - t_last; t_last = _t; } while (0)
#else
#define STAMP(i) do {} while (0)
#endif

template <typename T, int TAPS, int DIL>
__global__ void __launch_bounds__(256, TAPS == 1 ? 3 : 1)
conv_igemm_kernel(ConvKArgs a) {
#ifdef SEUNET_STAMP
  unsigned long long ph[12] = {0, 0, 0, 0, 0, 0, 0, 0, 0, 0, 0, 0};
  unsigned long long t_last = __builtin_readcyclecounter();
#endif
  constexpr int KC = Frag<T>::KC, KSTEPS = Frag<T>::KSTEPS;
  constexpr int HALO = (TAPS == 27) ? 1 : 0;
  constexpr int STEP = (TAPS == 27) ? DIL : 1;
  constexpr int HZ = CV_TZ + 2 * HALO, HY = CV_TY + 2 * HALO, HX = CV_TX + 2 * HALO;
  constexpr int NVH = HZ * HY * HX;
  constexpr int NCOL = 32;
  constexpr int T3 = (TAPS == 27) ? 3 : 1;
  constexpr int IN_ITEMS = (NVH * 2 + 255) / 256;
  constexpr int W_TOTAL = TAPS * NCOL * 2;
  constexpr int W_ITEMS = (W_TOTAL + 255) / 256;
  extern __shared__ __attribute__((aligned(16))) unsigned char smem[];
  unsigned char* in_tile = smem;
  unsigned char* w_tile = smem + IN_ITEMS * 4096 + 128;

  const int tid = threadIdx.x, lane = tid & 63, wave = tid >> 6;
  const int col = lane & 31, h = lane >> 5;
  int t;
  {
    const int nt = gridDim.x, b = blockIdx.x, q = nt >> 3, r = nt & 7, xcd = b & 7;
    t = (xcd < r ? xcd * (q + 1) : r * (q + 1) + (xcd - r) * q) + (b >> 3);
  }
  const int ntile = t % a.ncb;
  t /= a.ncb;
  const int tiles_per_sample = gridDim.x / a.ncb;
  const int tile_slot = t;
  const int bx = t % a.tx; t /= a.tx;
  const int by = t % a.ty; t /= a.ty;
  const int bz = t % a.tz;
  const int par = t / a.tz;
  const int px = par % STEP, py = (par / STEP) % STEP, pz = par / (STEP * STEP);
  const int x0 = bx * CV_TX, y0 = by * CV_TY, z0 = bz * CV_TZ;
  const int n = blockIdx.z;
  const long long V = (long long)a.D * a.H * a.W;

  const bool pair = a.pair != 0;
  const int piece = pair ? (lane & 1) : (wave & 1);
  const int vox0 = pair ? wave * 32 + (lane >> 1) : (wave >> 1) * 64 + lane;
  constexpr unsigned INVALID = 0xFFFFFFFFu;
  unsigned vofs[IN_ITEMS];
#pragma unroll
  for (int k = 0; k < IN_ITEMS; ++k) {
    const int vox = vox0 + 128 * k;
    const int hx = vox % HX;
    const int r2 = vox / HX;
    const int hy = r2 % HY, hz = r2 / HY;
    const int lz = z0 - HALO + hz, ly = y0 - HALO + hy, lx = x0 - HALO + hx;
    const int gz = STEP * lz + pz, gy = STEP * ly + py, gx = STEP * lx + px;
    const bool ok = vox < NVH && lz >= 0 && ly >= 0 && lx >= 0 && gz < a.D && gy < a.H && gx < a.W;
    vofs[k] = ok ? (unsigned)((gz * a.H + gy) * a.W + gx) : INVALID;
  }
  STAMP(8);
  constexpr int PLANE = IN_ITEMS * 2048 + 64;
  const int lds_in0 = piece * PLANE + vox0 * 16;
  const unsigned char* afrag0 = in_tile + (sizeof(T) == 2 ? h * PLANE : 4 * h) + (wave * HY * HX + col) * 16;
  const unsigned char* wfrag0 = w_tile + (h * NCOL + col) * (sizeof(T) == 2 ? 16 : 4);
  const unsigned char* wbase = reinterpret_cast<const unsigned char*>(a.wpack) +
                               (size_t)ntile * a.nchunks * (size_t)(W_TOTAL * 16);
  u32x4 rin[IN_ITEMS], rw[W_ITEMS];
  auto uniform_ptr = [](const void* p) -> const void* {
    const unsigned long long u = reinterpret_cast<unsigned long long>(p);
    const unsigned lo = __builtin_amdgcn_readfirstlane((unsigned)u), hi = __builtin_amdgcn_readfirstlane((unsigned)(u >> 32));
    return reinterpret_cast<const void*>(((unsigned long long)hi << 32) | lo);
  };
  __amdgpu_buffer_rsrc_t rs_in, rs_w;
  unsigned in_stride = 0;
  unsigned pofs = 0;
  bool pbad = false;
  auto fetch_setup = [&](int chunk) __attribute__((always_inline)) {
    const int chb = chunk * KC;
    const int ch0 = pair ? chb : chb + piece * (KC / 2);
    const void* sp = a.src0; int sC = a.srcC0, c = ch0;
    if (ch0 >= a.cum2) { sp = a.src2; sC = a.srcC2; c = ch0 - a.cum2; }
    else if (ch0 >= a.cum1) { sp = a.src1; sC = a.srcC1; c = ch0 - a.cum1; }
    const T* base = reinterpret_cast<const T*>(sp) + (long long)n * V * sC + c;
    const long long avail = ch0 < a.cin ? ((long long)V * sC - c) * (long long)sizeof(T) : 0;
    rs_in = __builtin_amdgcn_make_buffer_rsrc(const_cast<void*>(uniform_ptr(base)), 0,
                                              __builtin_amdgcn_readfirstlane((int)avail), RSRC_WORD3);
    in_stride = __builtin_amdgcn_readfirstlane((unsigned)(sC * (int)sizeof(T)));
    if (pair) {
      pofs = (unsigned)piece * 16u;
      pbad = piece == 1 && chb + KC / 2 >= a.cin;
    }
    rs_w = __builtin_amdgcn_make_buffer_rsrc(const_cast<void*>(uniform_ptr(wbase + (size_t)chunk * (W_TOTAL * 16))), 0,
                                             W_TOTAL * 16, RSRC_WORD3);
  };
  auto fetch_item = [&](auto item_c) __attribute__((always_inline)) {
    constexpr int item = decltype(item_c)::value;
    if constexpr (item < IN_ITEMS) {
      unsigned st = in_stride;
      asm volatile("" : "+s"(st));
      const unsigned off = pbad ? 0x80000000u : vofs[item] * st + pofs;
      rin[item] = __builtin_amdgcn_raw_buffer_load_b128(rs_in, off, 0, 0);
    } else if constexpr (item < IN_ITEMS + W_ITEMS) {
      constexpr int k = item - IN_ITEMS;
      rw[k] = __builtin_amdgcn_raw_buffer_load_b128(rs_w, (unsigned)tid * 16u, k * 4096, 0);
    }
  };
  constexpr int F_ITEMS = IN_ITEMS + W_ITEMS;

  f32x16 acc[4];
#pragma unroll
  for (int ms = 0; ms < 4; ++ms)
#pragma unroll
    for (int r = 0; r < 16; ++r) acc[ms][r] = 0.f;

  fetch_setup(0);
  static_for<F_ITEMS>([&](auto i_c) __attribute__((always_inline)) { fetch_item(i_c); });
  STAMP(0);
  for (int chunk = 0; chunk < a.nchunks; ++chunk) {
    __syncthreads();
    STAMP(1);
#pragma unroll
    for (int k = 0; k < IN_ITEMS; ++k) *reinterpret_cast<u32x4*>(in_tile + lds_in0 + k * 2048) = rin[k];
#pragma unroll
    for (int k = 0; k < W_ITEMS; ++k) *reinterpret_cast<u32x4*>(w_tile + (tid + 256 * k) * 16) = rw[k];
    STAMP(2);
    __syncthreads();
    STAMP(3);
    if (chunk + 1 < a.nchunks) {
      fetch_setup(chunk + 1);
      static_for<F_ITEMS>([&](auto i_c) __attribute__((always_inline)) { fetch_item(i_c); });
    }
    STAMP(4);

    {
      constexpr int NST = TAPS * KSTEPS;
      typedef typename std::conditional<sizeof(T) == 2, bf16x8, float>::type FragT;
      FragT wf[2], af[2][4];
      auto load_step = [&](auto st_c) __attribute__((always_inline)) {
        constexpr int st = decltype(st_c)::value;
        if constexpr (st < NST) {
          constexpr int tap = st / KSTEPS, ks = st % KSTEPS, b = st & 1;
          constexpr int tz3 = tap / (T3 * T3), ty3 = (tap / T3) % T3, tx3 = tap % T3;
          constexpr int voff = ((tz3 * HALO) * HY + ty3 * HALO) * HX + tx3 * HALO;
          if constexpr (sizeof(T) == 2) {
            wf[b] = *reinterpret_cast<const bf16x8*>(wfrag0 + tap * 2 * NCOL * 16);
#pragma unroll
            for (int ms = 0; ms < 4; ++ms)
              af[b][ms] = *reinterpret_cast<const bf16x8*>(afrag0 + (voff + ms * HX) * 16);
          } else {
            wf[b] = *reinterpret_cast<const float*>(wfrag0 + (tap * 4 + ks) * 2 * NCOL * 4);
#pragma unroll
            for (int ms = 0; ms < 4; ++ms)
              af[b][ms] = *reinterpret_cast<const float*>(afrag0 + (ks >> 1) * PLANE + 8 * (ks & 1) + (voff + ms * HX) * 16);
          }
        }
      };
      load_step(std::integral_constant<int, 0>{});
      static_for<NST>([&](auto st_c) __attribute__((always_inline)) {
        constexpr int ST = decltype(st_c)::value, b = ST & 1;
        load_step(std::integral_constant<int, ST + 1>{});
        __builtin_amdgcn_sched_barrier(0);
#pragma unroll
        for (int ms = 0; ms < 4; ++ms) {
          if constexpr (sizeof(T) == 2)
            acc[ms] = mfma_32x32x16<T>(wf[b], af[b][ms], acc[ms]);
          else
            acc[ms] = __builtin_amdgcn_mfma_f32_32x32x2f32(wf[b], af[b][ms], acc[ms], 0, 0, 0);
        }
        __builtin_amdgcn_sched_barrier(0);
      });
    }
    STAMP(5);
  }

  const int gz_w = STEP * (z0 + wave) + pz;
  const int gx_l = STEP * (x0 + col) + px;
  unsigned vlin[4];
  bool vok[4];
#pragma unroll
  for (int ms = 0; ms < 4; ++ms) {
    const int gy = STEP * (y0 + ms) + py;
    vok[ms] = gz_w < a.D && gy < a.H && gx_l < a.W;
    vlin[ms] = vok[ms] ? (unsigned)((gz_w * a.H + gy) * a.W + gx_l) : INVALID;
  }
  if (a.bias != nullptr) {
#pragma unroll
    for (int r = 0; r < 16; ++r) {
      const int co = ntile * NCOL + (r & 3) + 8 * (r >> 2) + 4 * h;
      const float bias = co < a.cout ? a.bias[co] : 0.f;
#pragma unroll
      for (int ms = 0; ms < 4; ++ms) acc[ms][r] += bias;
    }
  }
  constexpr int K_BYTES = (IN_ITEMS + W_ITEMS) * 4096 + 128;
  constexpr int E_BYTES = 4 * 128 * (NCOL * (int)sizeof(T) + 16);
  double* red = reinterpret_cast<double*>(smem + (K_BYTES > E_BYTES ? K_BYTES : E_BYTES));
  if (a.stats != nullptr) {
    float cntf = 0.f;
#pragma unroll
    for (int ms = 0; ms < 4; ++ms) cntf += vok[ms] ? 1.f : 0.f;
    cntf += dpp_fetch<0xB1>(cntf); cntf += dpp_fetch<0x4E>(cntf); cntf += dpp_fetch<0x141>(cntf); cntf += dpp_fetch<0x140>(cntf);
    cntf = dpp_settle(cntf);
    cntf += dpp_settle(__builtin_bit_cast(float, __builtin_amdgcn_ds_swizzle(__builtin_bit_cast(int, cntf), 0x401F)));
    const int j = col, rj = j & 15;
    typedef typename std::conditional<sizeof(T) == 4, double, float>::type R;
#pragma unroll
    for (int once = 0; once < 1; ++once) {
      float v0[16];
      R val[32];
#pragma unroll
      for (int r = 0; r < 16; ++r) {
        v0[r] = dpp_settle(__builtin_bit_cast(float, __builtin_amdgcn_ds_bpermute((lane & 32) * 4, __builtin_bit_cast(int, acc[0][r]))));
        R p1 = 0, p2 = 0;
#pragma unroll
        for (int ms = 0; ms < 4; ++ms) {
          const R dv = vok[ms] ? (R)acc[ms][r] - (R)v0[r] : (R)0;
          p1 += dv;
          p2 += dv * dv;
        }
        val[r] = p1; val[16 + r] = p2;
      }
      {
        const bool b4 = (j & 16) != 0, b3 = (j & 8) != 0, b2 = (j & 4) != 0, b1 = (j & 2) != 0, b0 = (j & 1) != 0;
#pragma unroll
        for (int i = 0; i < 16; ++i) {
          const R keep = b4 ? val[16 + i] : val[i], send = b4 ? val[i] : val[16 + i];
          val[i] = keep + xlane_swz16(send);
        }
#pragma unroll
        for (int i = 0; i < 8; ++i) {
          const R keep = b3 ? val[8 + i] : val[i], send = b3 ? val[i] : val[8 + i];
          val[i] = keep + xlane_dpp<0x128>(send);
        }
#pragma unroll
        for (int i = 0; i < 4; ++i) {
          const R keep = b2 ? val[4 + i] : val[i], send = b2 ? val[i] : val[4 + i];
          val[i] = keep + xlane_dpp<0x141>(send);
        }
#pragma unroll
        for (int i = 0; i < 2; ++i) {
          const R keep = b1 ? val[2 + i] : val[i], send = b1 ? val[i] : val[2 + i];
          val[i] = keep + xlane_dpp<0x4E>(send);
        }
        {
          const R keep = b0 ? val[1] : val[0], send = b0 ? val[0] : val[1];
          val[0] = keep + xlane_dpp<0xB1>(send);
        }
      }
      float sh = v0[0];
#pragma unroll
      for (int r = 1; r < 16; ++r) sh = (rj == r) ? v0[r] : sh;
      const R mine = dpp_settle(val[0]);
      const R s_of_q = xlane_swz16(mine);
      const double d0 = (double)sh, dc = (double)cntf;
      const double tot = j < 16 ? (double)mine + dc * d0
                                : (double)mine + 2.0 * d0 * (double)s_of_q + dc * d0 * d0;
      const int cl = (rj & 3) + 8 * (rj >> 2) + 4 * h;
      red[(wave * NCOL + cl) * 2 + (j >> 4)] = tot;
    }
  }
  STAMP(6);

  if (a.direct) {
    const int daccmask = a.dacc0 | (a.dacc1 << 1) | (a.dacc2 << 2);
    const int dC0 = a.dstC0, dC1 = a.dstC1, dC2 = a.dstC2;
    const unsigned long long dp0 = reinterpret_cast<unsigned long long>(a.dst0), dp1 = reinterpret_cast<unsigned long long>(a.dst1),
                             dp2 = reinterpret_cast<unsigned long long>(a.dst2);
#pragma unroll
    for (int once = 0; once < 1; ++once) {
#pragma unroll
      for (int q = 0; q < 4; ++q) {
        const int co8 = ntile * NCOL + 8 * q;
        if (co8 >= a.cout) continue;
        const int w1 = co8 >= a.dcum1 ? 1 : 0, w2 = co8 >= a.dcum2 ? 1 : 0;
        const int dC = dC0 + w1 * (dC1 - dC0) + w2 * (dC2 - dC1);
        const int cl = co8 - w1 * (a.dcum1 - w2 * a.dcum1) - w2 * a.dcum2;
        const int dacc = (daccmask >> (w1 + w2)) & 1;
        const unsigned long long dpu = dp0 + (unsigned long long)w1 * (dp1 - dp0) + (unsigned long long)w2 * (dp2 - dp1);
        void* dpv = reinterpret_cast<void*>(dpu);
        if (dpv == nullptr) continue;
        T* dbase = reinterpret_cast<T*>(dpv) + (long long)n * V * dC + cl;
        const long long davail = ((long long)V * dC - cl) * (long long)sizeof(T);
        const __amdgpu_buffer_rsrc_t rd = __builtin_amdgcn_make_buffer_rsrc(
            const_cast<void*>(uniform_ptr(dbase)), 0, __builtin_amdgcn_readfirstlane((int)davail), RSRC_WORD3);
        const unsigned dstride = __builtin_amdgcn_readfirstlane((unsigned)(dC * (int)sizeof(T)));
        const unsigned hofs = (unsigned)(4 * h * (int)sizeof(T));
#pragma unroll
        for (int ms = 0; ms < 4; ++ms) {
          const unsigned off = vok[ms] ? vlin[ms] * dstride + hofs : 0x80000000u;
          float v[4];
#pragma unroll
          for (int i = 0; i < 4; ++i) v[i] = acc[ms][4 * q + i];
          if constexpr (sizeof(T) == 2) {
            if (dacc) {
              const u32x2 o = __builtin_amdgcn_raw_buffer_load_b64(rd, off, 0, 0);
              v[0] += unpack_lo<T>(o.x); v[1] += unpack_hi<T>(o.x);
              v[2] += unpack_lo<T>(o.y); v[3] += unpack_hi<T>(o.y);
            }
            u32x2 u;
            u.x = pack2<T>(v[0], v[1]);
            u.y = pack2<T>(v[2], v[3]);
            __builtin_amdgcn_raw_buffer_store_b64(u, rd, off, 0, 0);
          } else {
            if (dacc) {
              const u32x4 o = __builtin_amdgcn_raw_buffer_load_b128(rd, off, 0, 0);
              v[0] += __uint_as_float(o.x); v[1] += __uint_as_float(o.y); v[2] += __uint_as_float(o.z); v[3] += __uint_as_float(o.w);
            }
            u32x4 u;
            u.x = __float_as_uint(v[0]); u.y = __float_as_uint(v[1]); u.z = __float_as_uint(v[2]); u.w = __float_as_uint(v[3]);
            __builtin_amdgcn_raw_buffer_store_b128(u, rd, off, 0, 0);
          }
        }
      }
    }
    STAMP(10);
  } else {
    __syncthreads();
    STAMP(7);
    constexpr int ROWB = NCOL * (int)sizeof(T) + 16;
    constexpr int PIECES = NCOL * (int)sizeof(T) / 16;
    constexpr int CPP = 16 / (int)sizeof(T);
    unsigned char* stage = smem + wave * (128 * ROWB);
#pragma unroll
    for (int ms = 0; ms < 4; ++ms)
#pragma unroll
      for (int q = 0; q < 4; ++q) {
        unsigned char* sp = stage + (ms * 32 + col) * ROWB + (8 * q + 4 * h) * (int)sizeof(T);
        if constexpr (sizeof(T) == 2) {
          u32x2 u;
          u.x = pack2<T>(acc[ms][4 * q], acc[ms][4 * q + 1]);
          u.y = pack2<T>(acc[ms][4 * q + 2], acc[ms][4 * q + 3]);
          *reinterpret_cast<u32x2*>(sp) = u;
        } else {
          u32x4 u;
          u.x = __float_as_uint(acc[ms][4 * q]); u.y = __float_as_uint(acc[ms][4 * q + 1]);
          u.z = __float_as_uint(acc[ms][4 * q + 2]); u.w = __float_as_uint(acc[ms][4 * q + 3]);
          *reinterpret_cast<u32x4*>(sp) = u;
        }
      }
    __builtin_amdgcn_wave_barrier();
    STAMP(9);
    {
      const int piece = lane % PIECES;
      const int co0 = ntile * NCOL + piece * CPP;
      T* sdst = nullptr; int sdC = 0, sdacc = 0;
      if (co0 < a.cout) {
        void* dpv = a.dst0; int cl = co0;
        sdC = a.dstC0; sdacc = a.dacc0;
        if (co0 >= a.dcum2) { dpv = a.dst2; sdC = a.dstC2; sdacc = a.dacc2; cl = co0 - a.dcum2; }
        else if (co0 >= a.dcum1) { dpv = a.dst1; sdC = a.dstC1; sdacc = a.dacc1; cl = co0 - a.dcum1; }
        if (dpv != nullptr) sdst = reinterpret_cast<T*>(dpv) + cl;
      }
#pragma unroll
      for (int i = 0; i < 2 * PIECES; ++i) {
        const int item = lane + 64 * i;
        const int vl = item / PIECES;
        const int gy = STEP * (y0 + (vl >> 5)) + py, gx = STEP * (x0 + (vl & 31)) + px;
        if (sdst != nullptr && gz_w < a.D && gy < a.H && gx < a.W) {
          u32x4 u = *reinterpret_cast<const u32x4*>(stage + vl * ROWB + piece * 16);
          u32x4* qp = reinterpret_cast<u32x4*>(sdst + ((long long)n * V + ((long long)gz_w * a.H + gy) * a.W + gx) * sdC);
          if (sdacc) {
            const u32x4 o = *qp;
            if constexpr (sizeof(T) == 2) {
#pragma unroll
              for (int e = 0; e < 4; ++e) {
                const float lo = unpack_lo<T>(u[e]) + unpack_lo<T>(o[e]);
                const float hi = unpack_hi<T>(u[e]) + unpack_hi<T>(o[e]);
                u[e] = pack2<T>(lo, hi);
              }
            } else {
#pragma unroll
              for (int e = 0; e < 4; ++e) u[e] = __float_as_uint(__uint_as_float(u[e]) + __uint_as_float(o[e]));
            }
          }
          *qp = u;
        }
      }
    }
    STAMP(10);

  }
  if (a.stats != nullptr) {
    asm volatile("s_waitcnt lgkmcnt(0)\n\ts_barrier" ::: "memory");
    if (tid < NCOL * 2) {
      const int c = tid >> 1, k = tid & 1;
      const int co = ntile * NCOL + c;
      if (co < a.cout) {
        const double tot = ((red[(0 * NCOL + c) * 2 + k] + red[(1 * NCOL + c) * 2 + k]) +
                            red[(2 * NCOL + c) * 2 + k]) + red[(3 * NCOL + c) * 2 + k];
        a.stats[(((long long)n * tiles_per_sample + tile_slot) * a.cout + co) * 2 + k] = tot;
      }
    }
  }
#ifdef SEUNET_STAMP
  STAMP(11);
  if (a.debug != nullptr && lane == 0) {
    const size_t w = (((size_t)blockIdx.z * gridDim.y + blockIdx.y) * gridDim.x + blockIdx.x) * 4 + wave;
    for (int i = 0; i < 12; ++i) a.debug[w * 12 + i] = ph[i];
  }
#endif
}

template <typename T>
__device__ __forceinline__ void conv_pack_body(const float* __restrict__ w, int taps, int cin_w, int cout_w, int tflip,
                                               T* __restrict__ out, int cin_e, int cout_e, int nchunks, int ncol,
                                               long long total) {
  constexpr int KC = Frag<T>::KC;
  for (long long i = blockIdx.x * (long long)blockDim.x + threadIdx.x; i < total;
       i += (long long)gridDim.x * blockDim.x) {
    long long r = i;
    int ci_in_chunk, col;
    if (sizeof(T) == 2) {
      const int j = (int)(r % 8); r /= 8;
      col = (int)(r % ncol); r /= ncol;
      const int hh = (int)(r % 2); r /= 2;
      ci_in_chunk = 8 * hh + j;
    } else {
      col = (int)(r % ncol); r /= ncol;
      const int hh = (int)(r % 2); r /= 2;
      const int ks = (int)(r % 4); r /= 4;
      ci_in_chunk = 2 * ks + hh;
    }
    const int tap = (int)(r % taps); r /= taps;
    const int chunk = (int)(r % nchunks);
    const int ntile = (int)(r / nchunks);
    const int ci = chunk * KC + ci_in_chunk, co = ntile * ncol + col;
    float v = 0.f;
    if (ci < cin_e && co < cout_e) {
      if (!tflip) v = w[((long long)co * cin_w + ci) * taps + tap];
      else v = w[((long long)ci * cin_w + co) * taps + (taps - 1 - tap)];
    }
    out[i] = from_f32<T>(v);
  }
}
template <typename T>
__global__ void conv_pack_kernel(const float* __restrict__ w, int taps, int cin_w, int cout_w, int tflip,
                                 T* __restrict__ out, int cin_e, int cout_e, int nchunks, int ncol,
                                 long long total) {
  conv_pack_body<T>(w, taps, cin_w, cout_w, tflip, out, cin_e, cout_e, nchunks, ncol, total);
}
struct PackEntry { const float* w; void* out; int taps, cin_w, cout_w, tflip, cin_e, cout_e, nchunks, ncol; long long total; };
struct PackList { PackEntry e[24]; };
template <typename T>
__global__ void conv_pack_multi_kernel(PackList l) {
  const PackEntry& e = l.e[blockIdx.y];
  conv_pack_body<T>(e.w, e.taps, e.cin_w, e.cout_w, e.tflip, reinterpret_cast<T*>(e.out), e.cin_e, e.cout_e, e.nchunks, e.ncol, e.total);
}

static constexpr int CV_NCOL = 32;
unsigned long long* g_conv_debug = nullptr;
static inline int conv_kc(int dtype) { return dtype_size(dtype) == 2 ? 16 : 8; }

size_t conv_wpack_bytes(int dtype, int taps, int cin, int cout) {
  const int ntiles = cdiv(cout, CV_NCOL), nchunks = cdiv(cin, conv_kc(dtype));
  return (size_t)ntiles * nchunks * taps * CV_NCOL * 32;
}

int launch_conv_pack_weights(int dtype, const float* w, int taps, int cin_w, int cout_w, int tflip,
                             void* wpack, hipStream_t s) {
  SEUNET_CHECK(taps == 27 || taps == 1, "conv pack: taps=%d unsupported", taps);
  const int cin_e = tflip ? cout_w : cin_w, cout_e = tflip ? cin_w : cout_w;
  const int nchunks = cdiv(cin_e, conv_kc(dtype));
  const long long total = (long long)(conv_wpack_bytes(dtype, taps, cin_e, cout_e) / dtype_size(dtype));
  const int grid = (int)((total + 255) / 256 > 4096 ? 4096 : (total + 255) / 256);
  SEUNET_DTYPE_SWITCH(dtype, conv_pack_kernel<T><<<grid, 256, 0, s>>>(w, taps, cin_w, cout_w, tflip, (T*)wpack, cin_e, cout_e, nchunks, CV_NCOL, total));
  SEUNET_LAUNCH_CHECK();
  return 0;
}

int launch_conv_pack_weights_multi(int dtype, const ConvPackJob* jobs, int n, hipStream_t s) {
  for (int base = 0; base < n; base += 24) {
    PackList l{};
    const int m = n - base < 24 ? n - base : 24;
    for (int i = 0; i < m; ++i) {
      const ConvPackJob& j = jobs[base + i];
      SEUNET_CHECK(j.taps == 27 || j.taps == 1, "conv pack: taps=%d unsupported", j.taps);
      PackEntry& e = l.e[i];
      e.w = j.w; e.out = j.wpack; e.taps = j.taps; e.cin_w = j.cin_w; e.cout_w = j.cout_w; e.tflip = j.tflip;
      e.cin_e = j.tflip ? j.cout_w : j.cin_w; e.cout_e = j.tflip ? j.cin_w : j.cout_w;
      e.ncol = CV_NCOL; e.nchunks = cdiv(e.cin_e, conv_kc(dtype));
      e.total = (long long)(conv_wpack_bytes(dtype, j.taps, e.cin_e, e.cout_e) / dtype_size(dtype));
    }
    SEUNET_DTYPE_SWITCH(dtype, conv_pack_multi_kernel<T><<<dim3(64, m), 256, 0, s>>>(l));
  }
  SEUNET_LAUNCH_CHECK();
  return 0;
}

int conv_stats_tiles(Dims d, int taps, int dil) {
  const int st = taps == 27 ? dil : 1;
  return cdiv(cdiv(d.D, st), CV_TZ) * cdiv(cdiv(d.H, st), CV_TY) * cdiv(cdiv(d.W, st), CV_TX) * st * st * st;
}

template <typename T, int TAPS, int DIL>
static int launch_one(const ConvKArgs& a, dim3 grid, hipStream_t s) {
  constexpr int HALO = (TAPS == 27) ? 1 : 0;
  constexpr int NVH = (CV_TZ + 2 * HALO) * (CV_TY + 2 * HALO) * (CV_TX + 2 * HALO);
  constexpr int LDS_K = ((NVH * 2 + 255) / 256 + (TAPS * 64 + 255) / 256) * 4096 + 128;
  constexpr int LDS_E = 4 * 128 * (32 * (int)sizeof(T) + 16);
  constexpr int LDS = (LDS_K > LDS_E ? LDS_K : LDS_E) + 4 * 32 * 16;
  static unsigned long long configured = 0;
  if (int e = configure_kernel_lds(configured, reinterpret_cast<const void*>(&conv_igemm_kernel<T, TAPS, DIL>), LDS)) return e;
  conv_igemm_kernel<T, TAPS, DIL><<<grid, 256, LDS, s>>>(a);
  SEUNET_LAUNCH_CHECK();
  return 0;
}

template <typename T>
static int launch_t(int taps, int dil, const ConvKArgs& a, dim3 grid, hipStream_t s) {
  if (taps == 1) return launch_one<T, 1, 1>(a, grid, s);
  if (dil == 1) return launch_one<T, 27, 1>(a, grid, s);
  return launch_one<T, 27, 2>(a, grid, s);
}

static int check_lists(const SrcList& src, const DstList& dst) {
  SEUNET_CHECK(src.n >= 1 && src.n <= 3 && dst.n >= 1 && dst.n <= 3, "conv: 1..3 sources/destinations");
  for (int i = 0; i < src.n; ++i)
    SEUNET_CHECK(src.C[i] > 0 && src.C[i] % 8 == 0 && src.ptr[i], "conv: source %d needs C %% 8 == 0 (got %d)", i, src.C[i]);
  for (int i = 0; i < dst.n; ++i)
    SEUNET_CHECK(dst.C[i] > 0 && dst.C[i] % 8 == 0, "conv: destination %d needs C %% 8 == 0 (got %d)", i, dst.C[i]);
  return 0;
}

int launch_conv_igemm(int dtype, int taps, int dil, const SrcList& src, int cin_logical, const void* wpack,
                      const float* bias, const DstList& dst, double* stats, Dims d, hipStream_t s) {
  if (int e = check_lists(src, dst)) return e;
  SEUNET_CHECK(cin_logical >= 1 && cin_logical <= src.total(), "conv: cin=%d exceeds the source channels %d", cin_logical, src.total());
  SEUNET_CHECK(taps == 27 || taps == 1, "conv: taps=%d unsupported", taps);
  SEUNET_CHECK(taps == 1 || dil == 1 || dil == 2, "conv: dilation %d unsupported", dil);
  ConvKArgs a{};
  a.src0 = src.ptr[0]; a.srcC0 = src.C[0];
  a.src1 = src.n > 1 ? src.ptr[1] : nullptr; a.srcC1 = src.n > 1 ? src.C[1] : 0;
  a.src2 = src.n > 2 ? src.ptr[2] : nullptr; a.srcC2 = src.n > 2 ? src.C[2] : 0;
  a.cin = cin_logical;
  a.cum1 = src.n > 1 ? src.C[0] : src.total();
  a.cum2 = src.n > 2 ? src.C[0] + src.C[1] : src.total();
  a.wpack = wpack; a.bias = bias;
  a.dst0 = dst.ptr[0]; a.dstC0 = dst.C[0]; a.dacc0 = dst.acc[0];
  a.dst1 = dst.n > 1 ? dst.ptr[1] : nullptr; a.dstC1 = dst.n > 1 ? dst.C[1] : 0; a.dacc1 = dst.n > 1 ? dst.acc[1] : 0;
  a.dst2 = dst.n > 2 ? dst.ptr[2] : nullptr; a.dstC2 = dst.n > 2 ? dst.C[2] : 0; a.dacc2 = dst.n > 2 ? dst.acc[2] : 0;
  a.cout = dst.total();
  a.dcum1 = dst.n > 1 ? dst.C[0] : a.cout;
  a.dcum2 = dst.n > 2 ? dst.C[0] + dst.C[1] : a.cout;
  a.stats = stats;
  a.N = d.N; a.D = d.D; a.H = d.H; a.W = d.W;
  const int st = taps == 27 ? dil : 1;
  a.tx = cdiv(cdiv(d.W, st), CV_TX); a.ty = cdiv(cdiv(d.H, st), CV_TY); a.tz = cdiv(cdiv(d.D, st), CV_TZ);
  a.nchunks = cdiv(a.cin, conv_kc(dtype));
  {
    const int kc = conv_kc(dtype);
    a.pair = (a.cum1 % kc == 0 || a.cum1 >= a.cin) && (a.cum2 % kc == 0 || a.cum2 >= a.cin) ? 1 : 0;
  }
  a.direct = 1;
  for (int i = 0; i < dst.n; ++i) if (dst.C[i] * st > 16) a.direct = 0;
  a.debug = g_conv_debug;
  a.ncb = cdiv(a.cout, CV_NCOL);
  dim3 grid(a.tx * a.ty * a.tz * st * st * st * a.ncb, 1, d.N);
  SEUNET_CHECK(d.N <= 65535, "conv: batch too large");
  for (int i = 0; i < src.n; ++i)
    SEUNET_CHECK((long long)d.vox() * src.C[i] * (long long)dtype_size(dtype) < (1LL << 31),
                 "conv: one sample of source %d is %lld bytes; the MFMA path addresses < 2^31 bytes per sample "
                 "(tile the volume, e.g. sliding_window_predict)", i, (long long)d.vox() * src.C[i] * (long long)dtype_size(dtype));
  for (int i = 0; i < dst.n; ++i)
    SEUNET_CHECK((long long)d.vox() * dst.C[i] * (long long)dtype_size(dtype) < (1LL << 31),
                 "conv: one sample of destination %d is %lld bytes; the MFMA path addresses < 2^31 bytes per sample",
                 i, (long long)d.vox() * dst.C[i] * (long long)dtype_size(dtype));
  SEUNET_DTYPE_SWITCH(dtype, return (launch_t<T>(taps, dil, a, grid, s)));
  return 1;
}

template <typename T>
__global__ void conv_naive_kernel(ConvKArgs a, const float* __restrict__ w, int taps, int dil, int tflip,
                                  int cin_w, long long total) {
  const long long V = (long long)a.D * a.H * a.W;
  const int t3 = taps == 27 ? 3 : 1, c = taps == 27 ? 1 : 0;
  for (long long i = blockIdx.x * (long long)blockDim.x + threadIdx.x; i < total;
       i += (long long)gridDim.x * blockDim.x) {
    const int co = (int)(i % a.cout);
    long long r = i / a.cout;
    const int x = (int)(r % a.W); r /= a.W;
    const int y = (int)(r % a.H); r /= a.H;
    const int z = (int)(r % a.D);
    const long long n = r / a.D;
    float acc = a.bias ? a.bias[co] : 0.f;
    for (int tap = 0; tap < taps; ++tap) {
      const int dz = (tap / (t3 * t3) - c) * dil, dy = ((tap / t3) % t3 - c) * dil, dx = (tap % t3 - c) * dil;
      const int zz = z + dz, yy = y + dy, xx = x + dx;
      if ((unsigned)zz >= (unsigned)a.D || (unsigned)yy >= (unsigned)a.H || (unsigned)xx >= (unsigned)a.W) continue;
      const long long vv = n * V + ((long long)zz * a.H + yy) * a.W + xx;
      for (int ci = 0; ci < a.cin; ++ci) {
        const void* sp = a.src0; int sC = a.srcC0, cc = ci;
        if (ci >= a.cum2) { sp = a.src2; sC = a.srcC2; cc = ci - a.cum2; }
        else if (ci >= a.cum1) { sp = a.src1; sC = a.srcC1; cc = ci - a.cum1; }
        const float xv = to_f32(reinterpret_cast<const T*>(sp)[vv * sC + cc]);
        const float wv = tflip ? w[((long long)ci * cin_w + co) * taps + (taps - 1 - tap)]
                               : w[((long long)co * cin_w + ci) * taps + tap];
        acc += xv * wv;
      }
    }
    void* dpv = a.dst0; int dC = a.dstC0, dacc = a.dacc0, cl = co;
    if (co >= a.dcum2) { dpv = a.dst2; dC = a.dstC2; dacc = a.dacc2; cl = co - a.dcum2; }
    else if (co >= a.dcum1) { dpv = a.dst1; dC = a.dstC1; dacc = a.dacc1; cl = co - a.dcum1; }
    if (dpv == nullptr) continue;
    T* q = reinterpret_cast<T*>(dpv) + (n * V + ((long long)z * a.H + y) * a.W + x) * dC + cl;
    if (dacc) acc += to_f32(*q);
    *q = from_f32<T>(acc);
  }
}

int launch_conv_naive(int dtype, int taps, int dil, const SrcList& src, int cin_logical, const float* w,
                      int tflip, const float* bias, const DstList& dst, Dims d, hipStream_t s) {
  if (int e = check_lists(src, dst)) return e;
  SEUNET_CHECK(cin_logical >= 1 && cin_logical <= src.total(), "conv: cin=%d exceeds the source channels %d", cin_logical, src.total());
  ConvKArgs a{};
  a.src0 = src.ptr[0]; a.srcC0 = src.C[0];
  a.src1 = src.n > 1 ? src.ptr[1] : nullptr; a.srcC1 = src.n > 1 ? src.C[1] : 0;
  a.src2 = src.n > 2 ? src.ptr[2] : nullptr; a.srcC2 = src.n > 2 ? src.C[2] : 0;
  a.cin = cin_logical;
  a.cum1 = src.n > 1 ? src.C[0] : src.total();
  a.cum2 = src.n > 2 ? src.C[0] + src.C[1] : src.total();
  a.bias = bias;
  a.dst0 = dst.ptr[0]; a.dstC0 = dst.C[0]; a.dacc0 = dst.acc[0];
  a.dst1 = dst.n > 1 ? dst.ptr[1] : nullptr; a.dstC1 = dst.n > 1 ? dst.C[1] : 0; a.dacc1 = dst.n > 1 ? dst.acc[1] : 0;
  a.dst2 = dst.n > 2 ? dst.ptr[2] : nullptr; a.dstC2 = dst.n > 2 ? dst.C[2] : 0; a.dacc2 = dst.n > 2 ? dst.acc[2] : 0;
  a.cout = dst.total();
  a.dcum1 = dst.n > 1 ? dst.C[0] : a.cout;
  a.dcum2 = dst.n > 2 ? dst.C[0] + dst.C[1] : a.cout;
  a.N = d.N; a.D = d.D; a.H = d.H; a.W = d.W;
  const long long total = (long long)d.N * d.vox() * a.cout;
  const int grid = (int)((total + 255) / 256 > 65535 ? 65535 : (total + 255) / 256);
  const int cin_w = tflip ? a.cout : cin_logical;
  SEUNET_DTYPE_SWITCH(dtype, conv_naive_kernel<T><<<grid, 256, 0, s>>>(a, w, taps, dil, tflip, cin_w, total));
  SEUNET_LAUNCH_CHECK();
  return 0;
}

}
```

### se-unet-airseg_amd/csrc/seunet_common.h

```cpp
#pragma once
#include <hip/hip_runtime.h>
#include <stdint.h>
#include <string>

#define SEUNET_F32 0
#define SEUNET_BF16 1
#define SEUNET_F16 2

typedef __bf16 bf16_t;
typedef _Float16 f16_t;

namespace seunet {

void set_error(const std::string& msg);
const char* get_error();
int fail(const char* fmt, ...);
bool prof_on();
void prof_mark(const char* tag, hipStream_t s);

#define SEUNET_CHECK(cond, ...)                       \
  do {                                                \
    if (!(cond)) return ::seunet::fail(__VA_ARGS__);  \
  } while (0)

#define SEUNET_HIP(expr)                                                              \
  do {                                                                                \
    hipError_t _e = (expr);                                                           \
    if (_e != hipSuccess)                                                             \
      return ::seunet::fail("%s failed: %s (%s:%d)", #expr, hipGetErrorString(_e),    \
                            __FILE__, __LINE__);                                      \
  } while (0)

#define SEUNET_LAUNCH_CHECK()                                                          \
  do {                                                                                \
    hipError_t _e = hipGetLastError();                                                \
    if (_e != hipSuccess)                                                             \
      return ::seunet::fail("kernel launch failed: %s (%s:%d)", hipGetErrorString(_e), \
                            __FILE__, __LINE__);                                      \
  } while (0)

static inline size_t dtype_size(int dtype) { return (dtype == SEUNET_BF16 || dtype == SEUNET_F16) ? 2 : 4; }
static inline bool dtype_ok(int dtype) { return dtype == SEUNET_F32 || dtype == SEUNET_BF16 || dtype == SEUNET_F16; }
#define SEUNET_DTYPE_SWITCH(DT, ...)                                   \
  do {                                                                 \
    if ((DT) == SEUNET_BF16) { typedef bf16_t T; __VA_ARGS__; }        \
    else if ((DT) == SEUNET_F16) { typedef f16_t T; __VA_ARGS__; }     \
    else { typedef float T; __VA_ARGS__; }                             \
  } while (0)
static inline int cdiv(int a, int b) { return (a + b - 1) / b; }
static inline size_t align_up(size_t v, size_t a) { return (v + a - 1) / a * a; }
static inline int grid_for(long long total, int block = 256) {
  long long g = (total + block - 1) / block;
  if (g > 256 * 16) g = 256 * 16;
  if (g < 1) g = 1;
  return (int)g;
}

struct Dims {
  int N, D, H, W;
  long long vox() const { return (long long)D * H * W; }
};

struct SrcList {
  const void* ptr[3];
  int C[3];
  int n;
  int total() const { int t = 0; for (int i = 0; i < n; ++i) t += C[i]; return t; }
  long long gap() const {
    return n < 2 ? 0 : reinterpret_cast<const unsigned char*>(ptr[1]) - reinterpret_cast<const unsigned char*>(ptr[0]);
  }
};

struct DstList {
  void* ptr[3];
  int C[3];
  int acc[3];
  int n;
  int total() const { int t = 0; for (int i = 0; i < n; ++i) t += C[i]; return t; }
};

#ifdef __HIPCC__
__device__ __forceinline__ float bf16_bits_to_f32(unsigned int hi16) {
  return __uint_as_float(hi16 << 16);
}
__device__ __forceinline__ unsigned int f32_to_bf16_bits(float f) {
  bf16_t b = (bf16_t)f;
  return (unsigned int)__builtin_bit_cast(unsigned short, b);
}
__device__ __forceinline__ float to_f32(float v) { return v; }
__device__ __forceinline__ float to_f32(bf16_t v) { return (float)v; }
__device__ __forceinline__ float to_f32(f16_t v) { return (float)v; }
template <typename T> __device__ __forceinline__ T from_f32(float v);
template <> __device__ __forceinline__ float from_f32<float>(float v) { return v; }
template <> __device__ __forceinline__ bf16_t from_f32<bf16_t>(float v) { return (bf16_t)v; }
template <> __device__ __forceinline__ f16_t from_f32<f16_t>(float v) { return (f16_t)v; }
template <typename T> __device__ __forceinline__ unsigned int pack2(float lo, float hi);
typedef float seunet_f32x2 __attribute__((ext_vector_type(2)));
typedef bf16_t seunet_bf16x2 __attribute__((ext_vector_type(2)));
typedef f16_t seunet_f16x2 __attribute__((ext_vector_type(2)));
template <> __device__ __forceinline__ unsigned int pack2<bf16_t>(float lo, float hi) {
  const seunet_f32x2 v = {lo, hi};
  return __builtin_bit_cast(unsigned int, __builtin_convertvector(v, seunet_bf16x2));
}
template <> __device__ __forceinline__ unsigned int pack2<f16_t>(float lo, float hi) {
  const seunet_f32x2 v = {lo, hi};
  return __builtin_bit_cast(unsigned int, __builtin_convertvector(v, seunet_f16x2));
}
template <typename T> __device__ __forceinline__ float unpack_lo(unsigned int u);
template <typename T> __device__ __forceinline__ float unpack_hi(unsigned int u);
template <> __device__ __forceinline__ float unpack_lo<bf16_t>(unsigned int u) { return bf16_bits_to_f32(u & 0xffffu); }
template <> __device__ __forceinline__ float unpack_hi<bf16_t>(unsigned int u) { return bf16_bits_to_f32(u >> 16); }
template <> __device__ __forceinline__ float unpack_lo<f16_t>(unsigned int u) { return (float)__builtin_bit_cast(f16_t, (unsigned short)(u & 0xffffu)); }
template <> __device__ __forceinline__ float unpack_hi<f16_t>(unsigned int u) { return (float)__builtin_bit_cast(f16_t, (unsigned short)(u >> 16)); }

__device__ __forceinline__ void load8(const float* p, float (&v)[8]) {
  const float4 a = reinterpret_cast<const float4*>(p)[0];
  const float4 b = reinterpret_cast<const float4*>(p)[1];
  v[0] = a.x; v[1] = a.y; v[2] = a.z; v[3] = a.w; v[4] = b.x; v[5] = b.y; v[6] = b.z; v[7] = b.w;
}
__device__ __forceinline__ void load8(const bf16_t* p, float (&v)[8]) {
  const uint4 u = *reinterpret_cast<const uint4*>(p);
  v[0] = bf16_bits_to_f32(u.x & 0xffffu); v[1] = bf16_bits_to_f32(u.x >> 16);
  v[2] = bf16_bits_to_f32(u.y & 0xffffu); v[3] = bf16_bits_to_f32(u.y >> 16);
  v[4] = bf16_bits_to_f32(u.z & 0xffffu); v[5] = bf16_bits_to_f32(u.z >> 16);
  v[6] = bf16_bits_to_f32(u.w & 0xffffu); v[7] = bf16_bits_to_f32(u.w >> 16);
}
__device__ __forceinline__ void load8(const f16_t* p, float (&v)[8]) {
  const uint4 u = *reinterpret_cast<const uint4*>(p);
  v[0] = unpack_lo<f16_t>(u.x); v[1] = unpack_hi<f16_t>(u.x); v[2] = unpack_lo<f16_t>(u.y); v[3] = unpack_hi<f16_t>(u.y);
  v[4] = unpack_lo<f16_t>(u.z); v[5] = unpack_hi<f16_t>(u.z); v[6] = unpack_lo<f16_t>(u.w); v[7] = unpack_hi<f16_t>(u.w);
}
__device__ __forceinline__ void store8(f16_t* p, const float (&v)[8]) {
  uint4 u;
  u.x = pack2<f16_t>(v[0], v[1]); u.y = pack2<f16_t>(v[2], v[3]); u.z = pack2<f16_t>(v[4], v[5]); u.w = pack2<f16_t>(v[6], v[7]);
  *reinterpret_cast<uint4*>(p) = u;
}
__device__ __forceinline__ void store8(float* p, const float (&v)[8]) {
  reinterpret_cast<float4*>(p)[0] = make_float4(v[0], v[1], v[2], v[3]);
  reinterpret_cast<float4*>(p)[1] = make_float4(v[4], v[5], v[6], v[7]);
}
__device__ __forceinline__ void store8(bf16_t* p, const float (&v)[8]) {
  uint4 u;
  u.x = pack2<bf16_t>(v[0], v[1]); u.y = pack2<bf16_t>(v[2], v[3]); u.z = pack2<bf16_t>(v[4], v[5]); u.w = pack2<bf16_t>(v[6], v[7]);
  *reinterpret_cast<uint4*>(p) = u;
}

template <typename T> struct Pack8;
template <> struct Pack8<bf16_t> { uint4 u; };
template <> struct Pack8<float> { float4 a, b; };
template <> struct Pack8<f16_t> { uint4 u; };
__device__ __forceinline__ void load8p(const f16_t* p, Pack8<f16_t>& k) { k.u = *reinterpret_cast<const uint4*>(p); }
__device__ __forceinline__ void unpack8(const Pack8<f16_t>& k, float (&v)[8]) {
  v[0] = unpack_lo<f16_t>(k.u.x); v[1] = unpack_hi<f16_t>(k.u.x); v[2] = unpack_lo<f16_t>(k.u.y); v[3] = unpack_hi<f16_t>(k.u.y);
  v[4] = unpack_lo<f16_t>(k.u.z); v[5] = unpack_hi<f16_t>(k.u.z); v[6] = unpack_lo<f16_t>(k.u.w); v[7] = unpack_hi<f16_t>(k.u.w);
}
__device__ __forceinline__ void zero8p(Pack8<f16_t>& k) { k.u = make_uint4(0, 0, 0, 0); }
__device__ __forceinline__ void load8p(const bf16_t* p, Pack8<bf16_t>& k) { k.u = *reinterpret_cast<const uint4*>(p); }
__device__ __forceinline__ void load8p(const float* p, Pack8<float>& k) {
  k.a = reinterpret_cast<const float4*>(p)[0];
  k.b = reinterpret_cast<const float4*>(p)[1];
}
__device__ __forceinline__ void unpack8(const Pack8<bf16_t>& k, float (&v)[8]) {
  v[0] = bf16_bits_to_f32(k.u.x & 0xffffu); v[1] = bf16_bits_to_f32(k.u.x >> 16);
  v[2] = bf16_bits_to_f32(k.u.y & 0xffffu); v[3] = bf16_bits_to_f32(k.u.y >> 16);
  v[4] = bf16_bits_to_f32(k.u.z & 0xffffu); v[5] = bf16_bits_to_f32(k.u.z >> 16);
  v[6] = bf16_bits_to_f32(k.u.w & 0xffffu); v[7] = bf16_bits_to_f32(k.u.w >> 16);
}
__device__ __forceinline__ void unpack8(const Pack8<float>& k, float (&v)[8]) {
  v[0] = k.a.x; v[1] = k.a.y; v[2] = k.a.z; v[3] = k.a.w; v[4] = k.b.x; v[5] = k.b.y; v[6] = k.b.z; v[7] = k.b.w;
}
__device__ __forceinline__ void zero8p(Pack8<bf16_t>& k) { k.u = make_uint4(0, 0, 0, 0); }
__device__ __forceinline__ void zero8p(Pack8<float>& k) { k.a = k.b = make_float4(0.f, 0.f, 0.f, 0.f); }

__device__ __forceinline__ int xcd_contiguous_tile(int b, int nt) {
  const int q = nt >> 3, r = nt & 7, xcd = b & 7;
  return (xcd < r ? xcd * (q + 1) : r * (q + 1) + (xcd - r) * q) + (b >> 3);
}
struct TileIdx3 { int x, y, z; };
__device__ __forceinline__ TileIdx3 xcd_contiguous_tile3() {
  const int b = (int)(blockIdx.x + gridDim.x * (blockIdx.y + gridDim.y * blockIdx.z));
  const int t = xcd_contiguous_tile(b, (int)(gridDim.x * gridDim.y * gridDim.z));
  TileIdx3 r;
  r.x = t % (int)gridDim.x;
  r.y = (t / (int)gridDim.x) % (int)gridDim.y;
  r.z = t / (int)(gridDim.x * gridDim.y);
  return r;
}
__device__ __forceinline__ float dpp_settle(float v) {
  asm volatile("v_mov_b32 %0, %0" : "+v"(v));
  return v;
}
__device__ __forceinline__ int dpp_settle(int v) {
  asm volatile("v_mov_b32 %0, %0" : "+v"(v));
  return v;
}
__device__ __forceinline__ unsigned long long dpp_settle(unsigned long long u) {
  unsigned lo = (unsigned)u, hi = (unsigned)(u >> 32);
  asm volatile("v_mov_b32 %0, %0\n\tv_mov_b32 %1, %1" : "+v"(lo), "+v"(hi));
  return ((unsigned long long)hi << 32) | lo;
}
__device__ __forceinline__ double dpp_settle(double v) {
  return __builtin_bit_cast(double, dpp_settle(__builtin_bit_cast(unsigned long long, v)));
}
template <typename V> __device__ __forceinline__ V shfl_xor_settled(V v, int off) { return dpp_settle(__shfl_xor(v, off, 64)); }
template <int CTRL> __device__ __forceinline__ int dpp_fetch_bits(int v) {
  return __builtin_amdgcn_update_dpp(0, v, CTRL, 0xF, 0xF, true);
}
template <int CTRL> __device__ __forceinline__ float dpp_fetch(float v) {
  return __builtin_bit_cast(float, dpp_fetch_bits<CTRL>(__builtin_bit_cast(int, v)));
}
template <int LPV> __device__ __forceinline__ float group_sum(float v) {
  static_assert(LPV == 1 || LPV == 2 || LPV == 4 || LPV == 8 || LPV == 16, "group_sum: LPV must be 1..16");
  if (LPV >= 2) v += dpp_fetch<0xB1>(v);
  if (LPV >= 4) v += dpp_fetch<0x4E>(v);
  if (LPV >= 8) v += dpp_fetch<0x141>(v);
  if (LPV >= 16) v += dpp_fetch<0x140>(v);
  return LPV >= 2 ? dpp_settle(v) : v;
}
template <int LPV> __device__ __forceinline__ float stride_sum(float v) {
#pragma unroll
  for (int off = 32; off >= LPV; off >>= 1) v += shfl_xor_settled(v, off);
  return v;
}
template <int LPV> __device__ __forceinline__ double stride_sum_d(double v) {
#pragma unroll
  for (int off = 32; off >= LPV; off >>= 1) v += shfl_xor_settled(v, off);
  return v;
}
#endif

int launch_pack_input(int dtype, const float* x_ncdhw, int in_channel, void* out_cl8, Dims d, hipStream_t s);
int launch_unpack_cl(int dtype, const void* in_cl, int C, float* out_ncdhw, Dims d, hipStream_t s);
int launch_pack_cl(int dtype, const float* in_ncdhw, int C, void* out_cl, int Cpad, Dims d, hipStream_t s);

size_t conv_wpack_bytes(int dtype, int taps, int cin, int cout);
int launch_conv_pack_weights(int dtype, const float* w_torch, int taps, int cin_w, int cout_w,
                             int transpose_flip, void* wpack, hipStream_t s);
int conv_stats_tiles(Dims d, int taps, int dil);
struct ConvPackJob { const float* w; void* wpack; int taps, cin_w, cout_w, tflip; };
int launch_conv_pack_weights_multi(int dtype, const ConvPackJob* jobs, int n, hipStream_t s);
int launch_conv_igemm(int dtype, int taps, int dil, const SrcList& src, int cin_logical,
                      const void* wpack, const float* bias, const DstList& dst,
                      double* stats_partial, Dims d, hipStream_t s);
int launch_conv_naive(int dtype, int taps, int dil, const SrcList& src, int cin_logical,
                      const float* w_torch, int transpose_flip, const float* bias,
                      const DstList& dst, Dims d, hipStream_t s);

bool conv_stream_supported(int dtype, int taps, int dil, int src_c, int dst_c);
size_t conv_stream_wpack_bytes(int src_c);
int conv_stream_slots(Dims d, int dil);
int launch_conv_stream_pack(int dtype, const float* w, int cin_w, int cout_w, int tflip, int src_c, int dst_c, void* wpack, hipStream_t s);
struct StreamPackJob { const float* w; void* wpack; int cin_w, cout_w, tflip, src_c, dst_c; };
int launch_conv_stream_pack_multi(int dtype, const StreamPackJob* jobs, int n, hipStream_t s);
int launch_conv_stream(int dtype, int dil, const void* src, int src_c, const void* wpack, const float* bias, void* dst, int dst_c,
                       int dst_accumulate, double* stats, Dims d, hipStream_t s);

bool conv_march_supported(int dtype, int taps, int dil, const SrcList& src, const DstList& dst);
size_t conv_march_wpack_bytes(int cin_e, int cout_e);
int conv_march_slots(Dims d, int dil, int cin_e, int cout_e);
int launch_conv_march_pack(int dtype, const float* w, int cin_w, int cout_w, int tflip, int cin_e, int cout_e, void* wpack, hipStream_t s);
struct MarchPackJob { const float* w; void* wpack; int cin_w, cout_w, tflip, cin_e, cout_e; };
int launch_conv_march_pack_multi(int dtype, const MarchPackJob* jobs, int n, hipStream_t s);
int launch_conv_march(int dtype, int dil, const SrcList& src, const void* wpack, const float* bias, const DstList& dst, double* stats,
                      Dims d, hipStream_t s);

bool wgrad_stream_supported(int dtype, int taps, int dil, int x_c, int dy_c);
size_t wgrad_stream_workspace_bytes(int x_c, int dy_c, int dil, Dims d);
int launch_wgrad_stream(int dtype, int dil, const void* x, int x_c, int cin_w, const void* dy, int dy_c, int cout_w, float* dw,
                        void* workspace, size_t ws_bytes, Dims d, hipStream_t s);

static constexpr int WG_TILED_SLABS = 512;
size_t wgrad_workspace_bytes(int taps, int cin, int cout);
int launch_wgrad(int dtype, int taps, int dil, const SrcList& x, int cin_logical, const void* dy,
                 int cout, float* dw_torch, void* workspace, size_t ws_bytes, Dims d, hipStream_t s);
bool wgrad_march_supported(int dtype, int taps, int dil, const SrcList& x, int cin_logical, int cout, Dims d, long long src_dist);
int launch_wgrad_march(int dtype, int taps, int dil, const SrcList& x, int cin_logical, const void* dy, int cout,
                       float* dw, void* workspace, size_t ws_bytes, Dims d, hipStream_t s);
size_t wgrad_march_workspace_bytes(int taps, int cin, int cout);
bool wgrad_1x1_supported(int dtype, const SrcList& x, int cin_logical, int cout);
int launch_wgrad_1x1(int dtype, const SrcList& x, int cin_logical, const void* dy, int cout, float* dw, void* workspace,
                     size_t ws_bytes, Dims d, hipStream_t s);
size_t wgrad_1x1_workspace_bytes(int cin, int cout);
int launch_wgrad_naive(int dtype, int taps, int dil, const SrcList& x, int cin_logical,
                       const void* dy, int cout, float* dw_torch, Dims d, hipStream_t s);
enum class ConvKernel { Naive, Tiled, Stream, March, Wgrad1x1 };
ConvKernel wgrad_kernel(int dtype, int taps, int dil, const SrcList& x, int cin_logical, int cout, Dims d, long long src_dist);
int run_wgrad(ConvKernel k, int dtype, int taps, int dil, const SrcList& x, int cin_logical, const void* dy, int cout, float* dw,
              void* workspace, size_t ws_bytes, Dims d, hipStream_t s);


int launch_xgrad_contract(int dtype, const void* d2, int C, const float* w2, int in_channel, float* gx, int accumulate, Dims d,
                          hipStream_t s);
int launch_xgrad_unpool(int dtype, const void* x_fine, int in_channel, const float* gx_coarse, float* gx_fine, Dims fine, hipStream_t s);
int launch_input_grad(int dtype, const void* draw, int ce, const float* w_ec1, const void* x0, int in_channel, const float* gx0,
                      const float* gx1, float* grad_x, Dims d, hipStream_t s);
int launch_maxpool_fwd(int dtype, const void* in, int C, void* out, Dims din, hipStream_t s);
int launch_maxpool_bwd(int dtype, const void* in, const void* g_out, int C, void* g_in,
                       int accumulate, Dims din, hipStream_t s);
int launch_upsample2_fwd(int dtype, const void* in, int C, void* out, Dims din, hipStream_t s);
int launch_upsample2_bwd(int dtype, const void* g_out, int C, void* g_in, int accumulate,
                         Dims din, hipStream_t s);
int upsample2_form(int dtype, int C, Dims din, bool backward);
int launch_multi_zero(float* const* ptrs, const int* counts, int n, hipStream_t s);
int class_max();
int class_grad_records(Dims d);
int launch_side_to_level(const float* side, const float* head_w, int wstride, const float* drop, int drop_stride, int K, float* level,
                         int accumulate, Dims d, hipStream_t s);
int launch_level_to_side_grad(const float* glev, long long cstride, long long nstride, const float* side, const float* head_w, int wstride,
                              const float* drop, int drop_stride, int K, float* g_side, double* partial, float* dhead, Dims d,
                              hipStream_t s);
int launch_class_bias_grad(const float* per_sample, int N, int K, float* out, hipStream_t s);
int launch_crop_batch(const void* img, int img_dtype, const unsigned char* label, const void* weight, int w_dtype,
                      const unsigned char* skel, int D, int H, int W, int cube, int ncrop, const int* starts, const int* aug,
                      double weight_exponent, int f64_math, float* data_out, float* label_out, float* weight_out, float* skel_out,
                      hipStream_t s);
int launch_hu_two_channel(const void* img, int img_dtype, long long nvox, int f64_math, float* out, hipStream_t s);
int launch_window_gather(const float* vol, int C, int X, int Y, int Z, int cube, int nwin, const int* starts, float* out, hipStream_t s);
int launch_window_accumulate(const float* logits, int apply_sigmoid, int nwin, const int* starts, int cube, double* acc, int X, int Y,
                             int Z, hipStream_t s);
int launch_window_finalize(const double* acc, int X, int Y, int Z, int cube, int nx, const int* xs, int ny, const int* ys, int nz,
                           const int* zs, int dup0, double* out, hipStream_t s);
int launch_adamw(float* const* params, const float* const* grads, float* const* exp_avg, float* const* exp_avg_sq,
                 const long long* counts, int n, double lr, double beta1, double beta2, double eps, double weight_decay,
                 int step, int maximize, hipStream_t s);
int configure_kernel_lds(unsigned long long& mask, const void* fn, int bytes);
const void* device_zero_page();
int launch_side_upsample(const float* side, int C, int scale, float* out_ncdhw, int c_total,
                         int c_off, Dims dlow, hipStream_t s);
int launch_head_fwd(const float* const* level_maps, int nlevels, const float* bias, float* pred,
                    Dims d0, hipStream_t s);
int launch_head_bwd(const float* g_pred, float* const* g_levels, int nlevels, float* tmp,
                    float* g_bias, Dims d0, hipStream_t s);
size_t head_bwd_tmp_floats(Dims d0);

#define SEUNET_LOSS_NSUMS 7
int loss_partials();
int launch_loss_sums(const float* pred, int apply_sigmoid, const float* target,
                     const float* weight, const float* skel, long long n, float* partial,
                     double* sums, hipStream_t s, int terms = 7);
int launch_loss_value(const double* sums0, double c_dice0, double c_gul0, double c_atr0, const double* sums1, double c_dice1,
                      double c_gul1, double c_atr1, float* value, hipStream_t s);
int launch_loss_grad(const float* pred, int apply_sigmoid, const float* target,
                     const float* weight, const float* skel, long long n, const double* sums,
                     float c_dice, float c_gul, float c_atr, float g_scale,
                     const float* g_scale_dev, float* g_pred, hipStream_t s);
int loss_sample_partials(int batch);
int launch_loss_sums_per_sample(const float* pred, int apply_sigmoid, const float* target, const float* weight, const float* skel,
                                int batch, long long n, float* partial, double* sums, int terms, hipStream_t s);
int launch_loss_sample_values(const double* sums, int batch, double c_dice, double c_gul, double c_atr, float* values, hipStream_t s);
#define SEUNET_POOL_MAX_CAPACITY 65535
#define SEUNET_POOL_MAX_BATCH 1024
#define SEUNET_POOL_MAX_GATHER 32
int launch_pool_select(const float* new_keys, int batch, float* keys, long long* seq, long long* state, int capacity, int* slots_out,
                       hipStream_t s);
int launch_pool_scatter(const int* slots_dev, int batch, int capacity, long long voxels, const float* data, const float* label,
                        const float* weight, const float* skel, float* pool_data, unsigned char* pool_label, float* pool_weight,
                        unsigned char* pool_skel, hipStream_t s);
int launch_pool_gather(const int* slots_host, int n, int capacity, long long voxels, const float* pool_data,
                       const unsigned char* pool_label, const float* pool_weight, const unsigned char* pool_skel, float* data_out,
                       float* label_out, float* weight_out, float* skel_out, hipStream_t s);
}
```

Before: 577.2 million.

## Add register-resident pointwise conv kernel looping over all output column blocks

Adds a dedicated 1x1x1 (pointwise) conv kernel for 16-bit dtypes. It keeps the whole input-channel slab for a voxel tile resident in registers and loops over every 32-wide output column block inside one workgroup, so inputs are loaded once rather than once per column block. The epilogue (bias, BN stats, store) is factored into a shared device function, and stats reduction scratch is double-buffered so the next block's weight load can overlap the current epilogue. It is selected only when there are at most 4 input chunks, more than one column block and enough tiles; the cost is fewer workgroups and higher register pressure.

Result: no change. 574.4 million (-0.5%).

```diff
diff --git a/include/seunet_hip.h b/include/seunet_hip.h
--- a/include/seunet_hip.h
+++ b/include/seunet_hip.h
@@ -32,6 +32,7 @@
 int seunet_conv3d_fwd(int dtype, int impl, int taps, int dilation, int nsrc, const void* const* src, const int* src_c,
                       int cin, const void* weights, int transpose_flip, const float* bias, int ndst, void* const* dst,
                       const int* dst_c, const int* dst_accumulate, double* stats_partial, seunet_dims dims, seunet_stream_t s);
+int seunet_conv3d_pointwise_form(int dtype, int nsrc, const int* src_c, int cin, int ndst, const int* dst_c, seunet_dims dims, int* out);
 int seunet_conv3d_stream_supported(int dtype, int dilation, int src_c, int dst_c);
 size_t seunet_conv3d_stream_wpack_bytes(int src_c);
 int seunet_conv3d_stream_slots(int dilation, seunet_dims dims);
diff --git a/se-unet-airseg_amd/_lib.py b/se-unet-airseg_amd/_lib.py
--- a/se-unet-airseg_amd/_lib.py
+++ b/se-unet-airseg_amd/_lib.py
@@ -51,6 +51,7 @@
     "seunet_conv_pack_weights": (_i, [_i, _vp, _i, _i, _i, _i, _vp, _vp]),
     "seunet_conv_stats_slots": (_i, [_i, _i, _i, Dims]),
     "seunet_conv3d_fwd": (_i, [_i, _i, _i, _i, _i, _pp, _ip, _i, _vp, _i, _vp, _i, _pp, _ip, _ip, _vp, Dims, _vp]),
+    "seunet_conv3d_pointwise_form": (_i, [_i, _i, _ip, _i, _i, _ip, Dims, _ip]),
     "seunet_conv3d_stream_supported": (_i, [_i, _i, _i, _i]),
     "seunet_conv3d_stream_wpack_bytes": (_sz, [_i]),
     "seunet_conv3d_stream_slots": (_i, [_i, Dims]),
diff --git a/se-unet-airseg_amd/csrc/abi.cpp b/se-unet-airseg_amd/csrc/abi.cpp
--- a/se-unet-airseg_amd/csrc/abi.cpp
+++ b/se-unet-airseg_amd/csrc/abi.cpp
@@ -101,6 +101,18 @@
   }
   return launch_conv_igemm(dtype, taps, dilation, sl, cin, weights, bias, dl, stats_partial, D(dims), S(s));
 }
+int seunet_conv3d_pointwise_form(int dtype, int nsrc, const int* src_c, int cin, int ndst, const int* dst_c, seunet_dims dims, int* out) {
+  SEUNET_CHECK(dtype_ok(dtype) && nsrc >= 1 && nsrc <= 3 && ndst >= 1 && ndst <= 3 && src_c && dst_c && out, "conv3d_pointwise_form: bad arguments");
+  int ctot = 0, cout = 0;
+  SrcList sl{};
+  sl.n = nsrc;
+  for (int i = 0; i < nsrc; ++i) { sl.C[i] = src_c[i]; ctot += src_c[i]; }
+  for (int i = 0; i < ndst; ++i) cout += dst_c[i];
+  SEUNET_CHECK(cin >= 1 && cin <= ctot && cout >= 1, "conv3d_pointwise_form: cin=%d exceeds the source channels %d", cin, ctot);
+  const PointwiseCut c = conv_pointwise_cut(dtype, sl, cin, cout, D(dims));
+  out[0] = c.regs; out[1] = c.resident; out[2] = c.ncb; out[3] = c.cpw; out[4] = c.grid_x;
+  return 0;
+}
 int seunet_conv3d_stream_supported(int dtype, int dilation, int src_c, int dst_c) { return conv_stream_supported(dtype, 27, dilation, src_c, dst_c) ? 1 : 0; }
 size_t seunet_conv3d_stream_wpack_bytes(int src_c) { return conv_stream_wpack_bytes(src_c); }
 int seunet_conv3d_stream_slots(int dilation, seunet_dims dims) { return conv_stream_slots(D(dims), dilation); }
diff --git a/se-unet-airseg_amd/csrc/conv_igemm.hip b/se-unet-airseg_amd/csrc/conv_igemm.hip
--- a/se-unet-airseg_amd/csrc/conv_igemm.hip
+++ b/se-unet-airseg_amd/csrc/conv_igemm.hip
@@ -25,6 +25,7 @@
   int pair;
   int direct;
   int ncb;
+  int cpw;
   unsigned long long* debug;
 };
 
@@ -52,9 +53,256 @@
 
 #ifdef SEUNET_STAMP
 #define STAMP(i) do { const unsigned long long _t = __builtin_readcyclecounter(); ph[i] += _t - t_last; t_last = _t; } while (0)
+#define STAMP_PARAMS , unsigned long long (&ph)[12], unsigned long long& t_last
+#define STAMP_ARGS , ph, t_last
 #else
 #define STAMP(i) do {} while (0)
+#define STAMP_PARAMS
+#define STAMP_ARGS
 #endif
+
+__device__ __forceinline__ const void* uniform_ptr(const void* p) {
+  const unsigned long long u = reinterpret_cast<unsigned long long>(p);
+  const unsigned lo = __builtin_amdgcn_readfirstlane((unsigned)u), hi = __builtin_amdgcn_readfirstlane((unsigned)(u >> 32));
+  return reinterpret_cast<const void*>(((unsigned long long)hi << 32) | lo);
+}
+__device__ __forceinline__ int xcd_contiguous(int b, int nt) {
+  const int q = nt >> 3, r = nt & 7, xcd = b & 7;
+  return (xcd < r ? xcd * (q + 1) : r * (q + 1) + (xcd - r) * q) + (b >> 3);
+}
+
+struct ConvTilePos {
+  int n, ntile, tile_slot, tiles_per_sample;
+  int x0, y0, z0, px, py, pz;
+};
+
+template <typename T, int STEP, bool KTILES>
+__device__ __forceinline__ void conv_epilogue(const ConvKArgs& a, f32x16 (&acc)[4], unsigned char* smem, double* red,
+                                              const ConvTilePos& p STAMP_PARAMS) {
+  constexpr int NCOL = 32;
+  constexpr unsigned INVALID = 0xFFFFFFFFu;
+  const int tid = threadIdx.x, lane = tid & 63, wave = tid >> 6;
+  const int col = lane & 31, h = lane >> 5;
+  const int n = p.n, ntile = p.ntile, tile_slot = p.tile_slot, tiles_per_sample = p.tiles_per_sample;
+  const int x0 = p.x0, y0 = p.y0, z0 = p.z0, px = p.px, py = p.py, pz = p.pz;
+  const long long V = (long long)a.D * a.H * a.W;
+  const int gz_w = STEP * (z0 + wave) + pz;
+  const int gx_l = STEP * (x0 + col) + px;
+  unsigned vlin[4];
+  bool vok[4];
+#pragma unroll
+  for (int ms = 0; ms < 4; ++ms) {
+    const int gy = STEP * (y0 + ms) + py;
+    vok[ms] = gz_w < a.D && gy < a.H && gx_l < a.W;
+    vlin[ms] = vok[ms] ? (unsigned)((gz_w * a.H + gy) * a.W + gx_l) : INVALID;
+  }
+  if (a.bias != nullptr) {
+#pragma unroll
+    for (int r = 0; r < 16; ++r) {
+      const int co = ntile * NCOL + (r & 3) + 8 * (r >> 2) + 4 * h;
+      const float bias = co < a.cout ? a.bias[co] : 0.f;
+#pragma unroll
+      for (int ms = 0; ms < 4; ++ms) acc[ms][r] += bias;
+    }
+  }
+  if (a.stats != nullptr) {
+    float cntf = 0.f;
+#pragma unroll
+    for (int ms = 0; ms < 4; ++ms) cntf += vok[ms] ? 1.f : 0.f;
+    cntf += dpp_fetch<0xB1>(cntf); cntf += dpp_fetch<0x4E>(cntf); cntf += dpp_fetch<0x141>(cntf); cntf += dpp_fetch<0x140>(cntf);
+    cntf = dpp_settle(cntf);
+    cntf += dpp_settle(__builtin_bit_cast(float, __builtin_amdgcn_ds_swizzle(__builtin_bit_cast(int, cntf), 0x401F)));
+    const int j = col, rj = j & 15;
+    typedef typename std::conditional<sizeof(T) == 4, double, float>::type R;
+#pragma unroll
+    for (int once = 0; once < 1; ++once) {
+      float v0[16];
+      R val[32];
+#pragma unroll
+      for (int r = 0; r < 16; ++r) {
+        v0[r] = dpp_settle(__builtin_bit_cast(float, __builtin_amdgcn_ds_bpermute((lane & 32) * 4, __builtin_bit_cast(int, acc[0][r]))));
+        R p1 = 0, p2 = 0;
+#pragma unroll
+        for (int ms = 0; ms < 4; ++ms) {
+          const R dv = vok[ms] ? (R)acc[ms][r] - (R)v0[r] : (R)0;
+          p1 += dv;
+          p2 += dv * dv;
+        }
+        val[r] = p1; val[16 + r] = p2;
+      }
+      {
+        const bool b4 = (j & 16) != 0, b3 = (j & 8) != 0, b2 = (j & 4) != 0, b1 = (j & 2) != 0, b0 = (j & 1) != 0;
+#pragma unroll
+        for (int i = 0; i < 16; ++i) {
+          const R keep = b4 ? val[16 + i] : val[i], send = b4 ? val[i] : val[16 + i];
+          val[i] = keep + xlane_swz16(send);
+        }
+#pragma unroll
+        for (int i = 0; i < 8; ++i) {
+          const R keep = b3 ? val[8 + i] : val[i], send = b3 ? val[i] : val[8 + i];
+          val[i] = keep + xlane_dpp<0x128>(send);
+        }
+#pragma unroll
+        for (int i = 0; i < 4; ++i) {
+          const R keep = b2 ? val[4 + i] : val[i], send = b2 ? val[i] : val[4 + i];
+          val[i] = keep + xlane_dpp<0x141>(send);
+        }
+#pragma unroll
+        for (int i = 0; i < 2; ++i) {
+          const R keep = b1 ? val[2 + i] : val[i], send = b1 ? val[i] : val[2 + i];
+          val[i] = keep + xlane_dpp<0x4E>(send);
+        }
+        {
+          const R keep = b0 ? val[1] : val[0], send = b0 ? val[0] : val[1];
+          val[0] = keep + xlane_dpp<0xB1>(send);
+        }
+      }
+      float sh = v0[0];
+#pragma unroll
+      for (int r = 1; r < 16; ++r) sh = (rj == r) ? v0[r] : sh;
+      const R mine = dpp_settle(val[0]);
+      const R s_of_q = xlane_swz16(mine);
+      const double d0 = (double)sh, dc = (double)cntf;
+      const double tot = j < 16 ? (double)mine + dc * d0
+                                : (double)mine + 2.0 * d0 * (double)s_of_q + dc * d0 * d0;
+      const int cl = (rj & 3) + 8 * (rj >> 2) + 4 * h;
+      red[(wave * NCOL + cl) * 2 + (j >> 4)] = tot;
+    }
+  }
+  STAMP(6);
+
+  if (a.direct) {
+    const int daccmask = a.dacc0 | (a.dacc1 << 1) | (a.dacc2 << 2);
+    const int dC0 = a.dstC0, dC1 = a.dstC1, dC2 = a.dstC2;
+    const unsigned long long dp0 = reinterpret_cast<unsigned long long>(a.dst0), dp1 = reinterpret_cast<unsigned long long>(a.dst1),
+                             dp2 = reinterpret_cast<unsigned long long>(a.dst2);
+#pragma unroll
+    for (int once = 0; once < 1; ++once) {
+#pragma unroll
+      for (int q = 0; q < 4; ++q) {
+        const int co8 = ntile * NCOL + 8 * q;
+        if (co8 >= a.cout) continue;
+        const int w1 = co8 >= a.dcum1 ? 1 : 0, w2 = co8 >= a.dcum2 ? 1 : 0;
+        const int dC = dC0 + w1 * (dC1 - dC0) + w2 * (dC2 - dC1);
+        const int cl = co8 - w1 * (a.dcum1 - w2 * a.dcum1) - w2 * a.dcum2;
+        const int dacc = (daccmask >> (w1 + w2)) & 1;
+        const unsigned long long dpu = dp0 + (unsigned long long)w1 * (dp1 - dp0) + (unsigned long long)w2 * (dp2 - dp1);
+        void* dpv = reinterpret_cast<void*>(dpu);
+        if (dpv == nullptr) continue;
+        T* dbase = reinterpret_cast<T*>(dpv) + (long long)n * V * dC + cl;
+        const long long davail = ((long long)V * dC - cl) * (long long)sizeof(T);
+        const __amdgpu_buffer_rsrc_t rd = __builtin_amdgcn_make_buffer_rsrc(
+            const_cast<void*>(uniform_ptr(dbase)), 0, __builtin_amdgcn_readfirstlane((int)davail), RSRC_WORD3);
+        const unsigned dstride = __builtin_amdgcn_readfirstlane((unsigned)(dC * (int)sizeof(T)));
+        const unsigned hofs = (unsigned)(4 * h * (int)sizeof(T));
+#pragma unroll
+        for (int ms = 0; ms < 4; ++ms) {
+          const unsigned off = vok[ms] ? vlin[ms] * dstride + hofs : 0x80000000u;
+          float v[4];
+#pragma unroll
+          for (int i = 0; i < 4; ++i) v[i] = acc[ms][4 * q + i];
+          if constexpr (sizeof(T) == 2) {
+            if (dacc) {
+              const u32x2 o = __builtin_amdgcn_raw_buffer_load_b64(rd, off, 0, 0);
+              v[0] += unpack_lo<T>(o.x); v[1] += unpack_hi<T>(o.x);
+              v[2] += unpack_lo<T>(o.y); v[3] += unpack_hi<T>(o.y);
+            }
+            u32x2 u;
+            u.x = pack2<T>(v[0], v[1]);
+            u.y = pack2<T>(v[2], v[3]);
+            __builtin_amdgcn_raw_buffer_store_b64(u, rd, off, 0, 0);
+          } else {
+            if (dacc) {
+              const u32x4 o = __builtin_amdgcn_raw_buffer_load_b128(rd, off, 0, 0);
+              v[0] += __uint_as_float(o.x); v[1] += __uint_as_float(o.y); v[2] += __uint_as_float(o.z); v[3] += __uint_as_float(o.w);
+            }
+            u32x4 u;
+            u.x = __float_as_uint(v[0]); u.y = __float_as_uint(v[1]); u.z = __float_as_uint(v[2]); u.w = __float_as_uint(v[3]);
+            __builtin_amdgcn_raw_buffer_store_b128(u, rd, off, 0, 0);
+          }
+        }
+      }
+    }
+    STAMP(10);
+  } else {
+    if constexpr (KTILES) __syncthreads();
+    STAMP(7);
+    constexpr int ROWB = NCOL * (int)sizeof(T) + 16;
+    constexpr int PIECES = NCOL * (int)sizeof(T) / 16;
+    constexpr int CPP = 16 / (int)sizeof(T);
+    unsigned char* stage = smem + wave * (128 * ROWB);
+#pragma unroll
+    for (int ms = 0; ms < 4; ++ms)
+#pragma unroll
+      for (int q = 0; q < 4; ++q) {
+        unsigned char* sp = stage + (ms * 32 + col) * ROWB + (8 * q + 4 * h) * (int)sizeof(T);
+        if constexpr (sizeof(T) == 2) {
+          u32x2 u;
+          u.x = pack2<T>(acc[ms][4 * q], acc[ms][4 * q + 1]);
+          u.y = pack2<T>(acc[ms][4 * q + 2], acc[ms][4 * q + 3]);
+          *reinterpret_cast<u32x2*>(sp) = u;
+        } else {
+          u32x4 u;
+          u.x = __float_as_uint(acc[ms][4 * q]); u.y = __float_as_uint(acc[ms][4 * q + 1]);
+          u.z = __float_as_uint(acc[ms][4 * q + 2]); u.w = __float_as_uint(acc[ms][4 * q + 3]);
+          *reinterpret_cast<u32x4*>(sp) = u;
+        }
+      }
+    __builtin_amdgcn_wave_barrier();
+    STAMP(9);
+    {
+      const int piece = lane % PIECES;
+      const int co0 = ntile * NCOL + piece * CPP;
+      T* sdst = nullptr; int sdC = 0, sdacc = 0;
+      if (co0 < a.cout) {
+        void* dpv = a.dst0; int cl = co0;
+        sdC = a.dstC0; sdacc = a.dacc0;
+        if (co0 >= a.dcum2) { dpv = a.dst2; sdC = a.dstC2; sdacc = a.dacc2; cl = co0 - a.dcum2; }
+        else if (co0 >= a.dcum1) { dpv = a.dst1; sdC = a.dstC1; sdacc = a.dacc1; cl = co0 - a.dcum1; }
+        if (dpv != nullptr) sdst = reinterpret_cast<T*>(dpv) + cl;
+      }
+#pragma unroll
+      for (int i = 0; i < 2 * PIECES; ++i) {
+        const int item = lane + 64 * i;
+        const int vl = item / PIECES;
+        const int gy = STEP * (y0 + (vl >> 5)) + py, gx = STEP * (x0 + (vl & 31)) + px;
+        if (sdst != nullptr && gz_w < a.D && gy < a.H && gx < a.W) {
+          u32x4 u = *reinterpret_cast<const u32x4*>(stage + vl * ROWB + piece * 16);
+          u32x4* qp = reinterpret_cast<u32x4*>(sdst + ((long long)n * V + ((long long)gz_w * a.H + gy) * a.W + gx) * sdC);
+          if (sdacc) {
+            const u32x4 o = *qp;
+            if constexpr (sizeof(T) == 2) {
+#pragma unroll
+              for (int e = 0; e < 4; ++e) {
+                const float lo = unpack_lo<T>(u[e]) + unpack_lo<T>(o[e]);
+                const float hi = unpack_hi<T>(u[e]) + unpack_hi<T>(o[e]);
+                u[e] = pack2<T>(lo, hi);
+              }
+            } else {
+#pragma unroll
+              for (int e = 0; e < 4; ++e) u[e] = __float_as_uint(__uint_as_float(u[e]) + __uint_as_float(o[e]));
+            }
+          }
+          *qp = u;
+        }
+      }
+    }
+    STAMP(10);
+
+  }
+  if (a.stats != nullptr) {
+    asm volatile("s_waitcnt lgkmcnt(0)\n\ts_barrier" ::: "memory");
+    if (tid < NCOL * 2) {
+      const int c = tid >> 1, k = tid & 1;
+      const int co = ntile * NCOL + c;
+      if (co < a.cout) {
+        const double tot = ((red[(0 * NCOL + c) * 2 + k] + red[(1 * NCOL + c) * 2 + k]) +
+                            red[(2 * NCOL + c) * 2 + k]) + red[(3 * NCOL + c) * 2 + k];
+        a.stats[(((long long)n * tiles_per_sample + tile_slot) * a.cout + co) * 2 + k] = tot;
+      }
+    }
+  }
+}
 
 template <typename T, int TAPS, int DIL>
 __global__ void __launch_bounds__(256, TAPS == 1 ? 3 : 1)
@@ -79,11 +327,7 @@
 
   const int tid = threadIdx.x, lane = tid & 63, wave = tid >> 6;
   const int col = lane & 31, h = lane >> 5;
-  int t;
-  {
-    const int nt = gridDim.x, b = blockIdx.x, q = nt >> 3, r = nt & 7, xcd = b & 7;
-    t = (xcd < r ? xcd * (q + 1) : r * (q + 1) + (xcd - r) * q) + (b >> 3);
-  }
+  int t = xcd_contiguous(blockIdx.x, gridDim.x);
   const int ntile = t % a.ncb;
   t /= a.ncb;
   const int tiles_per_sample = gridDim.x / a.ncb;
@@ -121,11 +365,6 @@
   const unsigned char* wbase = reinterpret_cast<const unsigned char*>(a.wpack) +
                                (size_t)ntile * a.nchunks * (size_t)(W_TOTAL * 16);
   u32x4 rin[IN_ITEMS], rw[W_ITEMS];
-  auto uniform_ptr = [](const void* p) -> const void* {
-    const unsigned long long u = reinterpret_cast<unsigned long long>(p);
-    const unsigned lo = __builtin_amdgcn_readfirstlane((unsigned)u), hi = __builtin_amdgcn_readfirstlane((unsigned)(u >> 32));
-    return reinterpret_cast<const void*>(((unsigned long long)hi << 32) | lo);
-  };
   __amdgpu_buffer_rsrc_t rs_in, rs_w;
   unsigned in_stride = 0;
   unsigned pofs = 0;
@@ -228,224 +467,119 @@
     STAMP(5);
   }
 
-  const int gz_w = STEP * (z0 + wave) + pz;
-  const int gx_l = STEP * (x0 + col) + px;
-  unsigned vlin[4];
-  bool vok[4];
-#pragma unroll
-  for (int ms = 0; ms < 4; ++ms) {
-    const int gy = STEP * (y0 + ms) + py;
-    vok[ms] = gz_w < a.D && gy < a.H && gx_l < a.W;
-    vlin[ms] = vok[ms] ? (unsigned)((gz_w * a.H + gy) * a.W + gx_l) : INVALID;
-  }
-  if (a.bias != nullptr) {
-#pragma unroll
-    for (int r = 0; r < 16; ++r) {
-      const int co = ntile * NCOL + (r & 3) + 8 * (r >> 2) + 4 * h;
-      const float bias = co < a.cout ? a.bias[co] : 0.f;
-#pragma unroll
-      for (int ms = 0; ms < 4; ++ms) acc[ms][r] += bias;
-    }
-  }
   constexpr int K_BYTES = (IN_ITEMS + W_ITEMS) * 4096 + 128;
   constexpr int E_BYTES = 4 * 128 * (NCOL * (int)sizeof(T) + 16);
   double* red = reinterpret_cast<double*>(smem + (K_BYTES > E_BYTES ? K_BYTES : E_BYTES));
-  if (a.stats != nullptr) {
-    float cntf = 0.f;
-#pragma unroll
-    for (int ms = 0; ms < 4; ++ms) cntf += vok[ms] ? 1.f : 0.f;
-    cntf += dpp_fetch<0xB1>(cntf); cntf += dpp_fetch<0x4E>(cntf); cntf += dpp_fetch<0x141>(cntf); cntf += dpp_fetch<0x140>(cntf);
-    cntf = dpp_settle(cntf);
-    cntf += dpp_settle(__builtin_bit_cast(float, __builtin_amdgcn_ds_swizzle(__builtin_bit_cast(int, cntf), 0x401F)));
-    const int j = col, rj = j & 15;
-    typedef typename std::conditional<sizeof(T) == 4, double, float>::type R;
-#pragma unroll
-    for (int once = 0; once < 1; ++once) {
-      float v0[16];
-      R val[32];
-#pragma unroll
-      for (int r = 0; r < 16; ++r) {
-        v0[r] = dpp_settle(__builtin_bit_cast(float, __builtin_amdgcn_ds_bpermute((lane & 32) * 4, __builtin_bit_cast(int, acc[0][r]))));
-        R p1 = 0, p2 = 0;
-#pragma unroll
-        for (int ms = 0; ms < 4; ++ms) {
-          const R dv = vok[ms] ? (R)acc[ms][r] - (R)v0[r] : (R)0;
-          p1 += dv;
-          p2 += dv * dv;
-        }
-        val[r] = p1; val[16 + r] = p2;
+  const ConvTilePos pos{n, ntile, tile_slot, tiles_per_sample, x0, y0, z0, px, py, pz};
+  conv_epilogue<T, STEP, true>(a, acc, smem, red, pos STAMP_ARGS);
+#ifdef SEUNET_STAMP
+  STAMP(11);
+  if (a.debug != nullptr && lane == 0) {
+    const size_t w = (((size_t)blockIdx.z * gridDim.y + blockIdx.y) * gridDim.x + blockIdx.x) * 4 + wave;
+    for (int i = 0; i < 12; ++i) a.debug[w * 12 + i] = ph[i];
+  }
+#endif
+}
+
+template <typename T, int RES>
+__global__ void __launch_bounds__(256, 2)
+conv_pointwise_kernel(ConvKArgs a) {
+  static_assert(sizeof(T) == 2, "the register form serves 16-bit storage");
+#ifdef SEUNET_STAMP
+  unsigned long long ph[12] = {0, 0, 0, 0, 0, 0, 0, 0, 0, 0, 0, 0};
+  unsigned long long t_last = __builtin_readcyclecounter();
+#endif
+  constexpr int KC = Frag<T>::KC, NCOL = 32;
+  constexpr unsigned INVALID = 0xFFFFFFFFu;
+  extern __shared__ __attribute__((aligned(16))) unsigned char smem[];
+  constexpr int E_BYTES = 4 * 128 * (NCOL * (int)sizeof(T) + 16);
+  double* red0 = reinterpret_cast<double*>(smem + E_BYTES);
+
+  const int tid = threadIdx.x, lane = tid & 63, wave = tid >> 6;
+  const int col = lane & 31, h = lane >> 5;
+  int t = xcd_contiguous(blockIdx.x, gridDim.x);
+  const int ngrp = a.ncb / a.cpw;
+  const int cb_begin = (t % ngrp) * a.cpw, cb_end = cb_begin + a.cpw;
+  t /= ngrp;
+  const int tiles_per_sample = gridDim.x / ngrp;
+  const int tile_slot = t;
+  const int bx = t % a.tx; t /= a.tx;
+  const int by = t % a.ty;
+  const int bz = t / a.ty;
+  const int x0 = bx * CV_TX, y0 = by * CV_TY, z0 = bz * CV_TZ;
+  const int n = blockIdx.z;
+  const long long V = (long long)a.D * a.H * a.W;
+
+  unsigned vofs[4];
+#pragma unroll
+  for (int ms = 0; ms < 4; ++ms) {
+    const int gz = z0 + wave, gy = y0 + ms, gx = x0 + col;
+    vofs[ms] = gz < a.D && gy < a.H && gx < a.W ? (unsigned)((gz * a.H + gy) * a.W + gx) : INVALID;
+  }
+  auto descriptor = [&](int ch, bool valid, unsigned& stride) __attribute__((always_inline)) {
+    const void* sp = a.src0; int sC = a.srcC0, c = ch;
+    if (ch >= a.cum2) { sp = a.src2; sC = a.srcC2; c = ch - a.cum2; }
+    else if (ch >= a.cum1) { sp = a.src1; sC = a.srcC1; c = ch - a.cum1; }
+    const T* base = reinterpret_cast<const T*>(sp) + (long long)n * V * sC + c;
+    const long long avail = valid ? ((long long)V * sC - c) * (long long)sizeof(T) : 0;
+    stride = __builtin_amdgcn_readfirstlane((unsigned)(sC * (int)sizeof(T)));
+    return __builtin_amdgcn_make_buffer_rsrc(const_cast<void*>(uniform_ptr(base)), 0,
+                                             __builtin_amdgcn_readfirstlane((int)avail), RSRC_WORD3);
+  };
+  const int xs = (a.cum1 % KC != 0 && a.cum1 < a.cin) ? a.cum1 / KC : (a.cum2 % KC != 0 && a.cum2 < a.cin) ? a.cum2 / KC : -1;
+  u32x4 bfr[RES][4], xfr[4], wfr[RES];
+  auto load_b = [&](int k0) __attribute__((always_inline)) {
+    static_for<RES>([&](auto c_c) __attribute__((always_inline)) {
+      constexpr int c = decltype(c_c)::value;
+      const int ch0 = (k0 + c) * KC, ch1 = ch0 + KC / 2;
+      const bool half = ch1 >= a.cin || k0 + c == xs;
+      unsigned st0;
+      const __amdgpu_buffer_rsrc_t rs0 = descriptor(ch0, k0 + c < a.nchunks, st0);
+      const unsigned out0 = 0u - ((unsigned)h & (half ? 1u : 0u));
+#pragma unroll
+      for (int ms = 0; ms < 4; ++ms)
+        bfr[c][ms] = __builtin_amdgcn_raw_buffer_load_b128(rs0, ((vofs[ms] * st0 + 16u * (unsigned)h) & ~out0) | (0x80000000u & out0), 0, 0);
+    });
+    unsigned st1;
+    const bool here = xs >= k0 && xs < k0 + RES;
+    const __amdgpu_buffer_rsrc_t rs1 = descriptor(here ? xs * KC + KC / 2 : 0, here, st1);
+    const unsigned out1 = 0u - ((unsigned)h ^ 1u);
+#pragma unroll
+    for (int ms = 0; ms < 4; ++ms)
+      xfr[ms] = __builtin_amdgcn_raw_buffer_load_b128(rs1, ((vofs[ms] * st1) & ~out1) | (0x80000000u & out1), 0, 0);
+  };
+  const __amdgpu_buffer_rsrc_t rs_w = __builtin_amdgcn_make_buffer_rsrc(
+      const_cast<void*>(uniform_ptr(a.wpack)), 0, __builtin_amdgcn_readfirstlane(a.ncb * a.nchunks * 1024), RSRC_WORD3);
+  auto load_w = [&](int cb, int k0) __attribute__((always_inline)) {
+    const int slab = __builtin_amdgcn_readfirstlane((cb * a.nchunks + k0) * 1024);
+    static_for<RES>([&](auto c_c) __attribute__((always_inline)) {
+      constexpr int c = decltype(c_c)::value;
+      wfr[c] = __builtin_amdgcn_raw_buffer_load_b128(rs_w, (unsigned)lane * 16u, slab + c * 1024, 0);
+    });
+  };
+
+  STAMP(8);
+  load_b(0);
+  load_w(cb_begin, 0);
+  for (int cb = cb_begin; cb < cb_end; ++cb) {
+    f32x16 acc[4];
+#pragma unroll
+    for (int ms = 0; ms < 4; ++ms)
+#pragma unroll
+      for (int r = 0; r < 16; ++r) acc[ms][r] = 0.f;
+    static_for<RES>([&](auto c_c) __attribute__((always_inline)) {
+      constexpr int c = decltype(c_c)::value;
+      if (c < a.nchunks) {
+        const unsigned both = c == xs ? 0xFFFFFFFFu : 0u;
+#pragma unroll
+        for (int ms = 0; ms < 4; ++ms)
+          acc[ms] = mfma_32x32x16<T>(__builtin_bit_cast(bf16x8, wfr[c]), __builtin_bit_cast(bf16x8, bfr[c][ms] | (xfr[ms] & both)), acc[ms]);
       }
-      {
-        const bool b4 = (j & 16) != 0, b3 = (j & 8) != 0, b2 = (j & 4) != 0, b1 = (j & 2) != 0, b0 = (j & 1) != 0;
-#pragma unroll
-        for (int i = 0; i < 16; ++i) {
-          const R keep = b4 ? val[16 + i] : val[i], send = b4 ? val[i] : val[16 + i];
-          val[i] = keep + xlane_swz16(send);
-        }
-#pragma unroll
-        for (int i = 0; i < 8; ++i) {
-          const R keep = b3 ? val[8 + i] : val[i], send = b3 ? val[i] : val[8 + i];
-          val[i] = keep + xlane_dpp<0x128>(send);
-        }
-#pragma unroll
-        for (int i = 0; i < 4; ++i) {
-          const R keep = b2 ? val[4 + i] : val[i], send = b2 ? val[i] : val[4 + i];
-          val[i] = keep + xlane_dpp<0x141>(send);
-        }
-#pragma unroll
-        for (int i = 0; i < 2; ++i) {
-          const R keep = b1 ? val[2 + i] : val[i], send = b1 ? val[i] : val[2 + i];
-          val[i] = keep + xlane_dpp<0x4E>(send);
-        }
-        {
-          const R keep = b0 ? val[1] : val[0], send = b0 ? val[0] : val[1];
-          val[0] = keep + xlane_dpp<0xB1>(send);
-        }
-      }
-      float sh = v0[0];
-#pragma unroll
-      for (int r = 1; r < 16; ++r) sh = (rj == r) ? v0[r] : sh;
-      const R mine = dpp_settle(val[0]);
-      const R s_of_q = xlane_swz16(mine);
-      const double d0 = (double)sh, dc = (double)cntf;
-      const double tot = j < 16 ? (double)mine + dc * d0
-                                : (double)mine + 2.0 * d0 * (double)s_of_q + dc * d0 * d0;
-      const int cl = (rj & 3) + 8 * (rj >> 2) + 4 * h;
-      red[(wave * NCOL + cl) * 2 + (j >> 4)] = tot;
-    }
-  }
-  STAMP(6);
-
-  if (a.direct) {
-    const int daccmask = a.dacc0 | (a.dacc1 << 1) | (a.dacc2 << 2);
-    const int dC0 = a.dstC0, dC1 = a.dstC1, dC2 = a.dstC2;
-    const unsigned long long dp0 = reinterpret_cast<unsigned long long>(a.dst0), dp1 = reinterpret_cast<unsigned long long>(a.dst1),
-                             dp2 = reinterpret_cast<unsigned long long>(a.dst2);
-#pragma unroll
-    for (int once = 0; once < 1; ++once) {
-#pragma unroll
-      for (int q = 0; q < 4; ++q) {
-        const int co8 = ntile * NCOL + 8 * q;
-        if (co8 >= a.cout) continue;
-        const int w1 = co8 >= a.dcum1 ? 1 : 0, w2 = co8 >= a.dcum2 ? 1 : 0;
-        const int dC = dC0 + w1 * (dC1 - dC0) + w2 * (dC2 - dC1);
-        const int cl = co8 - w1 * (a.dcum1 - w2 * a.dcum1) - w2 * a.dcum2;
-        const int dacc = (daccmask >> (w1 + w2)) & 1;
-        const unsigned long long dpu = dp0 + (unsigned long long)w1 * (dp1 - dp0) + (unsigned long long)w2 * (dp2 - dp1);
-        void* dpv = reinterpret_cast<void*>(dpu);
-        if (dpv == nullptr) continue;
-        T* dbase = reinterpret_cast<T*>(dpv) + (long long)n * V * dC + cl;
-        const long long davail = ((long long)V * dC - cl) * (long long)sizeof(T);
-        const __amdgpu_buffer_rsrc_t rd = __builtin_amdgcn_make_buffer_rsrc(
-            const_cast<void*>(uniform_ptr(dbase)), 0, __builtin_amdgcn_readfirstlane((int)davail), RSRC_WORD3);
-        const unsigned dstride = __builtin_amdgcn_readfirstlane((unsigned)(dC * (int)sizeof(T)));
-        const unsigned hofs = (unsigned)(4 * h * (int)sizeof(T));
-#pragma unroll
-        for (int ms = 0; ms < 4; ++ms) {
-          const unsigned off = vok[ms] ? vlin[ms] * dstride + hofs : 0x80000000u;
-          float v[4];
-#pragma unroll
-          for (int i = 0; i < 4; ++i) v[i] = acc[ms][4 * q + i];
-          if constexpr (sizeof(T) == 2) {
-            if (dacc) {
-              const u32x2 o = __builtin_amdgcn_raw_buffer_load_b64(rd, off, 0, 0);
-              v[0] += unpack_lo<T>(o.x); v[1] += unpack_hi<T>(o.x);
-              v[2] += unpack_lo<T>(o.y); v[3] += unpack_hi<T>(o.y);
-            }
-            u32x2 u;
-            u.x = pack2<T>(v[0], v[1]);
-            u.y = pack2<T>(v[2], v[3]);
-            __builtin_amdgcn_raw_buffer_store_b64(u, rd, off, 0, 0);
-          } else {
-            if (dacc) {
-              const u32x4 o = __builtin_amdgcn_raw_buffer_load_b128(rd, off, 0, 0);
-              v[0] += __uint_as_float(o.x); v[1] += __uint_as_float(o.y); v[2] += __uint_as_float(o.z); v[3] += __uint_as_float(o.w);
-            }
-            u32x4 u;
-            u.x = __float_as_uint(v[0]); u.y = __float_as_uint(v[1]); u.z = __float_as_uint(v[2]); u.w = __float_as_uint(v[3]);
-            __builtin_amdgcn_raw_buffer_store_b128(u, rd, off, 0, 0);
-          }
-        }
-      }
-    }
-    STAMP(10);
-  } else {
-    __syncthreads();
-    STAMP(7);
-    constexpr int ROWB = NCOL * (int)sizeof(T) + 16;
-    constexpr int PIECES = NCOL * (int)sizeof(T) / 16;
-    constexpr int CPP = 16 / (int)sizeof(T);
-    unsigned char* stage = smem + wave * (128 * ROWB);
-#pragma unroll
-    for (int ms = 0; ms < 4; ++ms)
-#pragma unroll
-      for (int q = 0; q < 4; ++q) {
-        unsigned char* sp = stage + (ms * 32 + col) * ROWB + (8 * q + 4 * h) * (int)sizeof(T);
-        if constexpr (sizeof(T) == 2) {
-          u32x2 u;
-          u.x = pack2<T>(acc[ms][4 * q], acc[ms][4 * q + 1]);
-          u.y = pack2<T>(acc[ms][4 * q + 2], acc[ms][4 * q + 3]);
-          *reinterpret_cast<u32x2*>(sp) = u;
-        } else {
-          u32x4 u;
-          u.x = __float_as_uint(acc[ms][4 * q]); u.y = __float_as_uint(acc[ms][4 * q + 1]);
-          u.z = __float_as_uint(acc[ms][4 * q + 2]); u.w = __float_as_uint(acc[ms][4 * q + 3]);
-          *reinterpret_cast<u32x4*>(sp) = u;
-        }
-      }
-    __builtin_amdgcn_wave_barrier();
-    STAMP(9);
-    {
-      const int piece = lane % PIECES;
-      const int co0 = ntile * NCOL + piece * CPP;
-      T* sdst = nullptr; int sdC = 0, sdacc = 0;
-      if (co0 < a.cout) {
-        void* dpv = a.dst0; int cl = co0;
-        sdC = a.dstC0; sdacc = a.dacc0;
-        if (co0 >= a.dcum2) { dpv = a.dst2; sdC = a.dstC2; sdacc = a.dacc2; cl = co0 - a.dcum2; }
-        else if (co0 >= a.dcum1) { dpv = a.dst1; sdC = a.dstC1; sdacc = a.dacc1; cl = co0 - a.dcum1; }
-        if (dpv != nullptr) sdst = reinterpret_cast<T*>(dpv) + cl;
-      }
-#pragma unroll
-      for (int i = 0; i < 2 * PIECES; ++i) {
-        const int item = lane + 64 * i;
-        const int vl = item / PIECES;
-        const int gy = STEP * (y0 + (vl >> 5)) + py, gx = STEP * (x0 + (vl & 31)) + px;
-        if (sdst != nullptr && gz_w < a.D && gy < a.H && gx < a.W) {
-          u32x4 u = *reinterpret_cast<const u32x4*>(stage + vl * ROWB + piece * 16);
-          u32x4* qp = reinterpret_cast<u32x4*>(sdst + ((long long)n * V + ((long long)gz_w * a.H + gy) * a.W + gx) * sdC);
-          if (sdacc) {
-            const u32x4 o = *qp;
-            if constexpr (sizeof(T) == 2) {
-#pragma unroll
-              for (int e = 0; e < 4; ++e) {
-                const float lo = unpack_lo<T>(u[e]) + unpack_lo<T>(o[e]);
-                const float hi = unpack_hi<T>(u[e]) + unpack_hi<T>(o[e]);
-                u[e] = pack2<T>(lo, hi);
-              }
-            } else {
-#pragma unroll
-              for (int e = 0; e < 4; ++e) u[e] = __float_as_uint(__uint_as_float(u[e]) + __uint_as_float(o[e]));
-            }
-          }
-          *qp = u;
-        }
-      }
-    }
-    STAMP(10);
-
-  }
-  if (a.stats != nullptr) {
-    asm volatile("s_waitcnt lgkmcnt(0)\n\ts_barrier" ::: "memory");
-    if (tid < NCOL * 2) {
-      const int c = tid >> 1, k = tid & 1;
-      const int co = ntile * NCOL + c;
-      if (co < a.cout) {
-        const double tot = ((red[(0 * NCOL + c) * 2 + k] + red[(1 * NCOL + c) * 2 + k]) +
-                            red[(2 * NCOL + c) * 2 + k]) + red[(3 * NCOL + c) * 2 + k];
-        a.stats[(((long long)n * tiles_per_sample + tile_slot) * a.cout + co) * 2 + k] = tot;
-      }
-    }
+    });
+    STAMP(5);
+    load_w(cb + 1, 0);
+    const ConvTilePos pos{n, cb, tile_slot, tiles_per_sample, x0, y0, z0, 0, 0, 0};
+    conv_epilogue<T, 1, false>(a, acc, smem, red0 + ((cb - cb_begin) & 1) * (4 * NCOL * 2), pos STAMP_ARGS);
   }
 #ifdef SEUNET_STAMP
   STAMP(11);
@@ -561,8 +695,37 @@
   return 0;
 }
 
+static constexpr int PW_RES = 4, PW_MIN_WG = 1024;
+PointwiseCut conv_pointwise_cut(int dtype, const SrcList& src, int cin, int cout, Dims d) {
+  PointwiseCut c;
+  int splits = 0;
+  for (int i = 0, cum = 0; i + 1 < src.n; ++i) {
+    cum += src.C[i];
+    if (cum % conv_kc(dtype) != 0 && cum < cin) ++splits;
+  }
+  c.tiles = conv_stats_tiles(d, 1, 1);
+  c.ncb = cdiv(cout, CV_NCOL);
+  const int nchunks = cdiv(cin, conv_kc(dtype));
+  c.regs = dtype_size(dtype) == 2 && splits <= 1 && c.ncb > 1 && nchunks <= PW_RES && (long long)c.tiles * d.N >= PW_MIN_WG ? 1 : 0;
+  c.resident = c.regs ? nchunks : 1;
+  c.cpw = c.regs ? c.ncb : 1;
+  c.grid_x = c.tiles * (c.ncb / c.cpw);
+  return c;
+}
+
+template <typename T, int RES>
+static int launch_pointwise(const ConvKArgs& a, dim3 grid, hipStream_t s) {
+  constexpr int LDS = 4 * 128 * (32 * (int)sizeof(T) + 16) + 2 * 4 * 32 * 16;
+  conv_pointwise_kernel<T, RES><<<grid, 256, LDS, s>>>(a);
+  SEUNET_LAUNCH_CHECK();
+  return 0;
+}
+
 template <typename T>
-static int launch_t(int taps, int dil, const ConvKArgs& a, dim3 grid, hipStream_t s) {
+static int launch_t(int taps, int dil, const ConvKArgs& a, dim3 grid, int regs, hipStream_t s) {
+  if constexpr (sizeof(T) == 2) {
+    if (regs) return launch_pointwise<T, PW_RES>(a, grid, s);
+  }
   if (taps == 1) return launch_one<T, 1, 1>(a, grid, s);
   if (dil == 1) return launch_one<T, 27, 1>(a, grid, s);
   return launch_one<T, 27, 2>(a, grid, s);
@@ -610,7 +773,15 @@
   for (int i = 0; i < dst.n; ++i) if (dst.C[i] * st > 16) a.direct = 0;
   a.debug = g_conv_debug;
   a.ncb = cdiv(a.cout, CV_NCOL);
+  a.cpw = 1;
   dim3 grid(a.tx * a.ty * a.tz * st * st * st * a.ncb, 1, d.N);
+  int regs = 0;
+  if (taps == 1) {
+    const PointwiseCut cut = conv_pointwise_cut(dtype, src, a.cin, a.cout, d);
+    regs = cut.regs;
+    a.cpw = cut.cpw;
+    grid.x = cut.grid_x;
+  }
   SEUNET_CHECK(d.N <= 65535, "conv: batch too large");
   for (int i = 0; i < src.n; ++i)
     SEUNET_CHECK((long long)d.vox() * src.C[i] * (long long)dtype_size(dtype) < (1LL << 31),
@@ -620,7 +791,7 @@
     SEUNET_CHECK((long long)d.vox() * dst.C[i] * (long long)dtype_size(dtype) < (1LL << 31),
                  "conv: one sample of destination %d is %lld bytes; the MFMA path addresses < 2^31 bytes per sample",
                  i, (long long)d.vox() * dst.C[i] * (long long)dtype_size(dtype));
-  SEUNET_DTYPE_SWITCH(dtype, return (launch_t<T>(taps, dil, a, grid, s)));
+  SEUNET_DTYPE_SWITCH(dtype, return (launch_t<T>(taps, dil, a, grid, regs, s)));
   return 1;
 }
 
diff --git a/se-unet-airseg_amd/csrc/seunet_common.h b/se-unet-airseg_amd/csrc/seunet_common.h
--- a/se-unet-airseg_amd/csrc/seunet_common.h
+++ b/se-unet-airseg_amd/csrc/seunet_common.h
@@ -237,6 +237,8 @@
 int launch_conv_pack_weights(int dtype, const float* w_torch, int taps, int cin_w, int cout_w,
                              int transpose_flip, void* wpack, hipStream_t s);
 int conv_stats_tiles(Dims d, int taps, int dil);
+struct PointwiseCut { int regs, resident, ncb, cpw, tiles, grid_x; };
+PointwiseCut conv_pointwise_cut(int dtype, const SrcList& src, int cin, int cout, Dims d);
 struct ConvPackJob { const float* w; void* wpack; int taps, cin_w, cout_w, tflip; };
 int launch_conv_pack_weights_multi(int dtype, const ConvPackJob* jobs, int n, hipStream_t s);
 int launch_conv_igemm(int dtype, int taps, int dil, const SrcList& src, int cin_logical,
```
